# facebookresearch/momentum

Measured on AMD Instinct MI355X. Metric: character IK solves/sec (72-joint, 10 GN iters), higher is better.
Workload: dtype f32; 1 GPU; BASELINE configs[1]: B x 72-joint humanoid, P=128, pos+ori on 16 landmarks (M=192), GN lambda=0.05, 10 it; batch_per_gpu=4096, global_batch=4096, joints=72, params=128, rows=192, solved_parameters=96, route=fused, line_search=0, precision=f32

## Files before the change

### include/mmx.h

```cpp
#ifndef MMX_H_
#define MMX_H_

#include <stddef.h>
#include <stdint.h>

#ifdef __cplusplus
extern "C" {
#endif

#define MMX_ABI_VERSION 12
#define MMX_PARAMS_PER_JOINT 7
#define MMX_INVALID_PARENT (-1)
#define MMX_MAX_MODEL_PARAMS 2048

typedef enum mmx_status {
  MMX_OK = 0,
  MMX_ERR_INVALID_ARGUMENT = 1,
  MMX_ERR_SIZE_MISMATCH = 2,
  MMX_ERR_DEVICE = 3,
  MMX_ERR_UNSUPPORTED = 4,
  MMX_ERR_OUT_OF_MEMORY = 5,
  MMX_ERR_NO_DEVICE = 6
} mmx_status;

// ... 136 lines not shown

typedef struct mmx_rig mmx_rig;
typedef struct mmx_problem mmx_problem;

void mmx_gn_options_default(mmx_gn_options* opt);

int32_t mmx_abi_version(void);
const char* mmx_last_error(void);
int32_t mmx_device_count(void);

int32_t mmx_rig_create(const mmx_rig_desc* desc, int32_t device, mmx_rig** out);
void mmx_rig_destroy(mmx_rig* rig);
int32_t mmx_rig_num_joints(const mmx_rig* rig);
int32_t mmx_rig_num_params(const mmx_rig* rig);

int32_t mmx_problem_create(
    mmx_rig* rig,
    int32_t batch,
    int32_t num_pos,
    const int32_t* pos_parent,
    int32_t num_ori,
    const int32_t* ori_parent,
    mmx_problem** out);
void mmx_problem_destroy(mmx_problem* problem);

int32_t mmx_problem_set_instance_rig(
    mmx_problem* problem,
    const float* translation_offset,
    const float* pre_rotation,
    int32_t memory,
    void* stream);

int32_t mmx_problem_set_instance_parents(
    mmx_problem* problem,
    const int32_t* pos_parent,
    const int32_t* ori_parent,
    int32_t memory,
    void* stream);

#define MMX_ROUTE_AUTO 0
#define MMX_ROUTE_FUSED 1
#define MMX_ROUTE_WIDE 2
#define MMX_ROUTE_EXPLICIT_JACOBIAN 3
#define MMX_ROUTE_WAVE 4
#define MMX_WAVE_MAX_JOINTS 64
#define MMX_WAVE_MAX_SOLVED 32
#define MMX_WAVE_MAX_UNITS 192
typedef struct mmx_tuning {
  int32_t route;
  int32_t max_refinement_steps;
  float mixed_tolerance;
  int32_t mixed_max_cg;
  int32_t joint_pruning;
  int32_t reserved[3];
} mmx_tuning;
int32_t mmx_problem_set_tuning(mmx_problem* problem, const mmx_tuning* tuning);
int32_t mmx_problem_last_route(const mmx_problem* problem);
int32_t mmx_problem_num_solve_joints(const mmx_problem* problem);

int32_t mmx_problem_num_rows(const mmx_problem* problem);
int32_t mmx_problem_batch(const mmx_problem* problem);

int32_t mmx_problem_set_enabled(mmx_problem* problem, const uint8_t* enabled);

int32_t mmx_problem_set_constraints(
    mmx_problem* problem,
    const mmx_constraint_data* data,
    void* stream);
int32_t mmx_problem_set_constraints_sized(
    mmx_problem* problem,
    const mmx_constraint_data* data,
    size_t data_size,
    void* stream);

int32_t mmx_eval_jacobian(
    mmx_problem* problem,
    const float* theta_dev,
    float* jac_dev,
    float* res_dev,
    double* err_dev,
    int32_t layout,
    void* stream);

int32_t mmx_eval_jacobian_timed(
    mmx_problem* problem,
    const float* theta_dev,
    float* jac_dev,
    float* res_dev,
    double* err_dev,
    int32_t layout,
    void* stream,
    float* kernel_ms);

int32_t mmx_debug_store_pattern(mmx_problem* problem, float* jac_dev, void* stream, float* kernel_ms);

int32_t mmx_eval_skeleton_state(
    mmx_problem* problem,
    const float* theta_dev,
    float* state_dev,
    void* stream);

int32_t mmx_eval_normal_equations(
    mmx_problem* problem,
    const float* theta_dev,
    float* jtj_dev,
    float* jtr_dev,
    double* err_dev,
    void* stream);

int32_t mmx_solve(
    mmx_problem* problem,
// ... 148 lines not shown
```

### momentum_amd/_abi.py

```python
from __future__ import annotations

import ctypes as C

import numpy as np

c_float_p = C.POINTER(C.c_float)
c_double_p = C.POINTER(C.c_double)
c_int32_p = C.POINTER(C.c_int32)
c_uint8_p = C.POINTER(C.c_uint8)

MMX_ABI_VERSION = 12
MMX_OK = 0
MMX_SOLVE_OK, MMX_SOLVE_NONFINITE, MMX_SOLVE_NOT_PD = 0, 1, 2
MMX_SOLVE_DAMPING_FLOORED = 4
MMX_SOLVE_PRECISION_SUSPECT = 8
MMX_SOLVE_ESCALATED_F64 = 16
MMX_SOLVE_MIXED = 32
MMX_SOLVE_ERROR_MASK = 3
MMX_PRECISION_F32, MMX_PRECISION_F64, MMX_PRECISION_AUTO, MMX_PRECISION_MIXED = 0, 1, 2, 3
MMX_MEM_HOST, MMX_MEM_DEVICE = 0, 1
MMX_LAYOUT_COL_MAJOR, MMX_LAYOUT_ROW_MAJOR = 0, 1
MMX_STEP_GN_FIXED_LAMBDA, MMX_STEP_LM_SCHEDULE, MMX_STEP_TRUST_REGION = 0, 1, 2


# ... 249 lines not shown
        ("do_line_search", C.c_int32),
        ("step_rule", C.c_int32),
        ("lm_lambda_min", C.c_float),
        ("lm_lambda_max", C.c_float),
        ("lm_up", C.c_float),
        ("lm_down", C.c_float),
        ("trust_region_radius", C.c_float),
        ("precision", C.c_int32),
        ("precision_bound", C.c_float),
    ]

    @classmethod
    def make(
        cls,
        min_iterations=1,
        max_iterations=2,
        threshold=1.0,
        regularization=0.05,
        do_line_search=False,
        step_rule=MMX_STEP_GN_FIXED_LAMBDA,
        lm_lambda_min=1e-6,
        lm_lambda_max=1e6,
        lm_up=4.0,
        lm_down=0.5,
        trust_region_radius=1.0,
        precision=MMX_PRECISION_F32,
        precision_bound=1e-5,
    ) -> "GnOptions":
        return cls(
            int(min_iterations),
            int(max_iterations),
            float(threshold),
            float(regularization),
            int(do_line_search),
            int(step_rule),
            float(lm_lambda_min),
            float(lm_lambda_max),
            float(lm_up),
            float(lm_down),
            float(trust_region_radius),
            int(precision),
            float(precision_bound),
        )


ROUTES = {"auto": 0, "fused": 1, "wide": 2, "explicit_jacobian": 3, "wave": 4}
WAVE_MAX_JOINTS = 64
WAVE_MAX_SOLVED = 32
WAVE_MAX_UNITS = 192


class Tuning(C.Structure):

    _fields_ = [("route", C.c_int32), ("max_refinement_steps", C.c_int32), ("mixed_tolerance", C.c_float), ("mixed_max_cg", C.c_int32), ("joint_pruning", C.c_int32), ("reserved", C.c_int32 * 3)]


def as_ptr(a: np.ndarray, ctype):
    assert a.flags["C_CONTIGUOUS"], "array must be C-contiguous"
    return a.ctypes.data_as(C.POINTER(ctype))


def void_p(a) -> C.c_void_p:
    if a is None:
        return C.c_void_p(0)
    if isinstance(a, np.ndarray):
        assert a.flags["C_CONTIGUOUS"]
        return C.c_void_p(a.ctypes.data)
    return C.c_void_p(int(a))
```

### momentum_amd/build.py

```python
from __future__ import annotations

import os
import shutil
import subprocess
import sys

HERE = os.path.dirname(os.path.abspath(__file__))
CSRC = os.path.join(HERE, "csrc")
VARIANT = os.environ.get("MMX_BUILD_VARIANT", "")
VARIANT_FLAGS = os.environ.get("MMX_BUILD_FLAGS", "").split() if VARIANT else []
LIB = os.path.join(HERE, f"libmmx_hip_{VARIANT}.so" if VARIANT else "libmmx_hip.so")
SOURCES = ["mmx_kernels.hip", "mmx_fused.hip", "mmx_capi.hip", "mmx_comm.hip", "mmx_f64.hip", "mmx_host_tables.cpp", "mmx_solve_plan.cpp", "mmx_constraint_intake.cpp", "mmx_wave.hip", "mmx_wave_frames.hip", "mmx_gradient.hip"]
FUSED_GROUPS = 7
SOLVE_KERNEL_FLAGS = ["-mllvm", "-disable-machine-licm", "-mllvm", "-disable-lsr"]
BUILD_INFO = os.path.join(HERE, "build_info.json")
_probe_cache = {}


def solve_flags_accepted() -> bool:
    if os.environ.get("MMX_BUILD_DEFAULT_PIPELINE"):
        return False
    if "ok" not in _probe_cache:
        import tempfile

        with tempfile.TemporaryDirectory() as td:
            src = os.path.join(td, "probe.hip")
            with open(src, "w") as f:
                f.write("#include <hip/hip_runtime.h>\n__global__ void k(float* p) { for (int i = 0; i < 8; ++i) p[i * 3] += 1.f; }\n")
            cmd = [_hipcc(), f"--offload-arch={ARCH}", "-O3", "-c", src, "-o", os.path.join(td, "probe.o")] + SOLVE_KERNEL_FLAGS
            r = subprocess.run(cmd, stdout=subprocess.PIPE, stderr=subprocess.PIPE)
            _probe_cache["ok"] = r.returncode == 0
            if r.returncode != 0:
                print(
                    "WARNING momentum_amd/build.py: hipcc rejects " + " ".join(SOLVE_KERNEL_FLAGS) + " -- the solve kernels are built with the "
                    "DEFAULT pipeline (they spill vector registers and run 6-13 % slower; build_info.json says so):\n" + r.stderr.decode(errors="replace")[-400:],
                    file=sys.stderr,
                )
    return _probe_cache["ok"]


def _wants_solve_flags(src: str, group) -> bool:
    return src in ("mmx_f64.hip",) or (src == "mmx_fused.hip" and group != 4)


def _extra_flags(src: str, group) -> list:
    if _wants_solve_flags(src, group):
        return SOLVE_KERNEL_FLAGS
    return []


def build_info() -> dict:
    import json

    try:
        with open(BUILD_INFO) as f:
            return json.load(f)
    except (OSError, ValueError):
        return {}
SOURCE_DEPS = {"mmx_wave_frames.hip": ["mmx_wave.hip"]}
HEADERS = ["mmx_device.hpp", "mmx_device_d.hpp", "mmx_kernels.hpp", "mmx_tree.hpp", "mmx_fused_helpers.hpp", "mmx_host_tables.hpp", "mmx_solve_plan.hpp", "mmx_constraint_intake.hpp", os.path.join("..", "..", "include", "mmx.h")]
ARCH = "gfx950"


def _hipcc() -> str:
    for cand in (shutil.which("hipcc"), "/opt/rocm/bin/hipcc"):
        if cand and os.path.exists(cand):
            return cand
    raise RuntimeError("hipcc not found (ROCm toolchain required to build the gfx950 kernels)")


def needs_build() -> bool:
    if not os.path.exists(LIB) or (not VARIANT and not os.path.exists(BUILD_INFO)):
        return True
    t = os.path.getmtime(LIB)
    deps = [os.path.join(CSRC, s) for s in SOURCES + HEADERS]
    return any(os.path.getmtime(d) > t for d in deps)


def build(force: bool = False, verbose: bool = False) -> str:
    if not force and not needs_build():
        return LIB
    jobs, keep = [], []
    flags_ok = solve_flags_accepted()
    hdr_time = max(os.path.getmtime(os.path.join(CSRC, h)) for h in HEADERS)
    for src in SOURCES:
        groups = range(FUSED_GROUPS) if src == "mmx_fused.hip" else [None]
        for g in groups:
            stem = os.path.splitext(src)[0] + ("" if g is None else f"_g{g}")
            obj = os.path.join(CSRC, stem + (f".{VARIANT}" if VARIANT else "") + ".o")
            cmd = [_hipcc(), f"--offload-arch={ARCH}", "-O3", "-std=c++17", "-fPIC", "-c", os.path.join(CSRC, src), "-o", obj]
            if VARIANT:
                cmd.insert(1, f"-DMMX_EXP_{VARIANT.upper()}")
                cmd[1:1] = VARIANT_FLAGS
            if g is not None:
                cmd.insert(1, f"-DMMX_FUSED_GROUP={g}")
            if flags_ok:
                cmd[1:1] = _extra_flags(src, g)
            if src.endswith(".cpp"):
                cmd.insert(1, "-x")
                cmd.insert(2, "hip")
            src_time = max(os.path.getmtime(os.path.join(CSRC, d)) for d in [src] + SOURCE_DEPS.get(src, []))
            if not force and os.path.exists(obj) and os.path.getmtime(obj) > max(hdr_time, src_time):
                keep.append((None, obj))
                continue
            jobs.append((cmd, obj))
    from concurrent.futures import ThreadPoolExecutor

    def run(job):
        if verbose:
            print(" ".join(job[0]), file=sys.stderr)
        subprocess.check_call(job[0])
        return job[1]

# ... 35 lines not shown
```

### momentum_amd/capi.py

```python
from __future__ import annotations

import ctypes as C
import os
from typing import Optional

import numpy as np

from . import _abi
from ._abi import ConstraintData, GnOptions, RigDesc, as_ptr
from .rigs import Rig

_HERE = os.path.dirname(os.path.abspath(__file__))
LIB_PATH = os.environ.get("MMX_LIB") or os.path.join(_HERE, "libmmx_hip.so")
_lib: Optional[C.CDLL] = None

SYMBOLS = [
    "mmx_gn_options_default", "mmx_abi_version", "mmx_last_error", "mmx_device_count",
    "mmx_rig_create", "mmx_rig_destroy", "mmx_rig_num_joints", "mmx_rig_num_params",
    "mmx_problem_create", "mmx_problem_destroy", "mmx_problem_num_rows", "mmx_problem_batch",
    "mmx_problem_set_tuning", "mmx_problem_last_route", "mmx_problem_num_solve_joints",
    "mmx_problem_set_enabled", "mmx_problem_set_constraints", "mmx_problem_set_constraints_sized", "mmx_problem_set_instance_rig", "mmx_problem_set_instance_parents", "mmx_eval_jacobian", "mmx_eval_jacobian_timed", "mmx_debug_store_pattern",
    "mmx_eval_skeleton_state", "mmx_eval_normal_equations", "mmx_solve", "mmx_solve_with_history", "mmx_solve_with_step_history", "mmx_problem_solve_diagnostics", "mmx_solve_f64", "mmx_solve_f64_host", "mmx_solve_host",
    "mmx_solve_frames", "mmx_solve_frames_host",
    "mmx_eval_gradient", "mmx_eval_gradient_host",
    "mmx_eval_jacobian_host", "mmx_eval_skeleton_state_host", "mmx_host_tables", "mmx_debug_fused_normal_equations", "mmx_debug_tree_normal_equations",
    "mmx_host_elimination_order", "mmx_host_tile_structure", "mmx_host_tile_level_schedule", "mmx_host_f64_assembly_list", "mmx_problem_tile_structure", "mmx_host_live_joints",
    "mmx_comm_unique_id", "mmx_comm_create", "mmx_comm_create_all", "mmx_comm_world_size", "mmx_comm_rank",
    "mmx_comm_all_reduce_norms", "mmx_comm_all_reduce_norms_host", "mmx_residual_norms", "mmx_comm_destroy",
]


class MmxError(RuntimeError):

    def __init__(self, code: int, msg: str):
        super().__init__(f"mmx error {code}: {msg}")
        self.code = code


def lib() -> C.CDLL:
    global _lib
    if _lib is not None:
        return _lib
    if not os.path.exists(LIB_PATH):
        raise MmxError(-1, f"{LIB_PATH} is missing: build it with `python -m momentum_amd.build` (no CPU fallback exists)")
    try:
        import torch
    except Exception:
        pass
    L = C.CDLL(LIB_PATH)
    vp, i32 = C.c_void_p, C.c_int32
    L.mmx_last_error.restype = C.c_char_p
    L.mmx_gn_options_default.restype = None
    L.mmx_gn_options_default.argtypes = [C.POINTER(GnOptions)]
    L.mmx_rig_create.argtypes = [C.POINTER(RigDesc), i32, C.POINTER(vp)]
    L.mmx_rig_destroy.argtypes = [vp]
    L.mmx_rig_destroy.restype = None
    L.mmx_rig_num_joints.argtypes = [vp]
    L.mmx_rig_num_params.argtypes = [vp]
    L.mmx_problem_create.argtypes = [vp, i32, i32, _abi.c_int32_p, i32, _abi.c_int32_p, C.POINTER(vp)]
    L.mmx_problem_destroy.argtypes = [vp]
    L.mmx_problem_destroy.restype = None
    L.mmx_problem_num_rows.argtypes = [vp]
    L.mmx_problem_batch.argtypes = [vp]
    L.mmx_problem_set_enabled.argtypes = [vp, _abi.c_uint8_p]
    L.mmx_problem_set_tuning.argtypes = [vp, C.POINTER(_abi.Tuning)]
    L.mmx_problem_last_route.argtypes = [vp]
    L.mmx_problem_num_solve_joints.argtypes = [vp]
    L.mmx_problem_set_constraints.argtypes = [vp, C.POINTER(ConstraintData), vp]
    L.mmx_problem_set_constraints_sized.argtypes = [vp, C.POINTER(ConstraintData), C.c_size_t, vp]
    L.mmx_problem_set_instance_rig.argtypes = [vp, vp, vp, i32, vp]
    L.mmx_problem_set_instance_parents.argtypes = [vp, vp, vp, i32, vp]
    L.mmx_eval_jacobian.argtypes = [vp, vp, vp, vp, vp, i32, vp]
    L.mmx_eval_jacobian_timed.argtypes = [vp, vp, vp, vp, vp, i32, vp, C.POINTER(C.c_float)]
    L.mmx_debug_store_pattern.argtypes = [vp, vp, vp, C.POINTER(C.c_float)]
    L.mmx_eval_skeleton_state.argtypes = [vp, vp, vp, vp]
    L.mmx_eval_normal_equations.argtypes = [vp, vp, vp, vp, vp, vp]
    L.mmx_solve.argtypes = [vp, C.POINTER(GnOptions), vp, vp, vp, vp, vp, vp]
    L.mmx_solve_with_history.argtypes = [vp, C.POINTER(GnOptions), vp, vp, vp, vp, vp, vp, vp]
    L.mmx_solve_with_step_history.argtypes = [vp, C.POINTER(GnOptions), vp, vp, vp, vp, vp, vp, vp, vp]
    L.mmx_problem_solve_diagnostics.argtypes = [vp, vp, vp]
    L.mmx_solve_f64.argtypes = [vp, C.POINTER(GnOptions), vp, vp, vp, vp, vp, vp]
    L.mmx_solve_host.argtypes = [vp, C.POINTER(GnOptions), vp, vp, vp, vp]
    L.mmx_solve_f64_host.argtypes = [vp, C.POINTER(GnOptions), vp, vp, vp, vp]
    L.mmx_solve_frames.argtypes = [vp, C.POINTER(GnOptions), i32, vp, vp, vp, vp, vp, vp, vp]
    L.mmx_solve_frames_host.argtypes = [vp, C.POINTER(GnOptions), i32, vp, vp, vp, vp]
    L.mmx_eval_gradient.argtypes = [vp, vp, vp, vp, vp]
    L.mmx_eval_gradient_host.argtypes = [vp, vp, vp, vp]
    L.mmx_eval_jacobian_host.argtypes = [vp, vp, vp, vp, vp, i32]
    L.mmx_eval_skeleton_state_host.argtypes = [vp, vp, vp]
    L.mmx_debug_tree_normal_equations.argtypes = [vp, vp, vp, vp, vp]
    L.mmx_debug_fused_normal_equations.argtypes = [vp, vp, vp, vp, _abi.c_int32_p, _abi.c_int32_p, vp]
    L.mmx_comm_unique_id.argtypes = [vp]
    L.mmx_comm_create.argtypes = [vp, i32, i32, i32, C.POINTER(vp)]
    L.mmx_comm_create_all.argtypes = [i32, _abi.c_int32_p, C.POINTER(vp)]
    L.mmx_comm_world_size.argtypes = [vp]
    L.mmx_comm_rank.argtypes = [vp]
    L.mmx_comm_all_reduce_norms.argtypes = [vp, vp, vp]
    L.mmx_comm_all_reduce_norms_host.argtypes = [vp, vp]
    L.mmx_residual_norms.argtypes = [i32, vp, vp, vp, vp, vp]
    L.mmx_comm_destroy.argtypes = [vp]
    L.mmx_comm_destroy.restype = None
    L.mmx_host_tables.argtypes = [
        C.POINTER(RigDesc), _abi.c_uint8_p, _abi.c_int32_p, _abi.c_int32_p, _abi.c_int32_p,
        _abi.c_uint8_p, _abi.c_int32_p, _abi.c_int32_p,
    ]
    u32p, i64p = C.POINTER(C.c_uint32), C.POINTER(C.c_int64)
    L.mmx_host_elimination_order.argtypes = [C.POINTER(RigDesc), _abi.c_uint8_p, _abi.c_int32_p, _abi.c_int32_p]
    L.mmx_host_tile_structure.argtypes = [i32, _abi.c_uint8_p, u32p, u32p, i64p]
    L.mmx_host_tile_level_schedule.argtypes = [i32, _abi.c_uint8_p, C.POINTER(C.c_int32)]
    L.mmx_problem_tile_structure.argtypes = [vp, u32p, u32p, _abi.c_int32_p, _abi.c_int32_p, i64p]
    L.mmx_host_live_joints.argtypes = [C.POINTER(RigDesc), i32, _abi.c_int32_p, _abi.c_uint8_p, _abi.c_int32_p, _abi.c_int32_p]
    _lib = L
    return L


def _check(rc: int) -> None:
    if rc != 0:
        raise MmxError(rc, lib().mmx_last_error().decode("utf-8", "replace"))


# ... 117 lines not shown


default_route = "auto"


class Problem:

    def __init__(self, rig_handle: RigHandle, batch: int, pos_parent, ori_parent):
        import torch

        self.rh = rig_handle
        self.B = int(batch)
        self.P = rig_handle.rig.num_params
        self.J = rig_handle.rig.num_joints
        self.pos_parent = np.ascontiguousarray(pos_parent, dtype=np.int32).reshape(-1)
        self.ori_parent = np.ascontiguousarray(ori_parent, dtype=np.int32).reshape(-1)
        self.Kp, self.Ko = len(self.pos_parent), len(self.ori_parent)
        self.M = 3 * self.Kp + 9 * self.Ko
        self.n = self.P
        self.device = torch.device("cuda", rig_handle.device)
        self._h = C.c_void_p(0)
        self._keep = []
        _check(
            lib().mmx_problem_create(
                rig_handle._h, self.B, self.Kp, as_ptr(self.pos_parent, C.c_int32), self.Ko,
                as_ptr(self.ori_parent, C.c_int32), C.byref(self._h),
            )
        )
        self._prefer_wide = default_route == "prefer_wide"
        if default_route not in ("auto", "prefer_wide"):
            self.set_route(default_route)

    def close(self) -> None:
        if self._h:
            lib().mmx_problem_destroy(self._h)
            self._h = C.c_void_p(0)

    def __del__(self):
        try:
            self.close()
        except Exception:
            pass

    def set_route(self, route: str, max_refinement_steps: int = 0) -> None:
        self._prefer_wide = default_route == "prefer_wide" and route == "auto"
        self._set_tuning(route, max_refinement_steps)

    def _set_tuning(self, route: str, max_refinement_steps: int = 0) -> None:
        t = _abi.Tuning()
        t.route = _abi.ROUTES[route]
        t.max_refinement_steps = int(max_refinement_steps)
        t.mixed_tolerance, t.mixed_max_cg = getattr(self, "_mixed", (0.0, 0))
        t.joint_pruning = 0 if getattr(self, "_joint_pruning", True) else -1
        self._route_args = (route, int(max_refinement_steps))
        _check(lib().mmx_problem_set_tuning(self._h, C.byref(t)))

    def set_mixed(self, tolerance: float = 0.0, max_cg: int = 0) -> None:
        self._mixed = (float(tolerance), int(max_cg))
        self._set_tuning(*getattr(self, "_route_args", ("auto", 0)))

    def set_joint_pruning(self, on: bool = True) -> None:
        self._joint_pruning = bool(on)
        self._set_tuning(*getattr(self, "_route_args", ("auto", 0)))

    def num_solve_joints(self) -> int:
        return int(lib().mmx_problem_num_solve_joints(self._h))

    def last_route(self) -> str:
        r = int(lib().mmx_problem_last_route(self._h))
        return {v: k for k, v in _abi.ROUTES.items()}[r]

    def set_enabled(self, enabled) -> None:
        e = np.ascontiguousarray(enabled, dtype=np.uint8).reshape(-1)
        assert e.shape[0] == self.P
        _check(lib().mmx_problem_set_enabled(self._h, as_ptr(e, C.c_uint8)))
        self.n = int(np.count_nonzero(e))

    def set_constraints(
        self, pos_offset, pos_target, pos_weight, ori_offset, ori_target, ori_weight,
        pos_function_weight: float = 1.0, ori_function_weight: float = 1.0,
        limits=None, limit_function_weight: float = 1.0,
        model_target=None, model_weights=None, model_function_weight: float = 1.0,
        pos_loss=(2.0, 1.0), ori_loss=(2.0, 1.0), joint_blocks=None, ellipsoid_limits=None, function_weights=None,
    ) -> None:
        import torch

        arrs = [pos_offset, pos_target, pos_weight, ori_offset, ori_target, ori_weight]
        shapes = [(self.B, self.Kp, 3), (self.B, self.Kp, 3), (self.B, self.Kp), (self.B, self.Ko, 4), (self.B, self.Ko, 4), (self.B, self.Ko)]
        if model_target is not None:
            arrs += [model_target, model_weights]
            shapes += [(self.B, self.P), (self.B, self.P)]
        on_dev = all(isinstance(a, torch.Tensor) for a in arrs)
        keep, ptrs = [], []
        for a, shp in zip(arrs, shapes):
            if on_dev:
                assert a.is_cuda and a.dtype == torch.float32 and a.is_contiguous() and tuple(a.shape) == shp, (a.shape, shp)
                keep.append(a)
                ptrs.append(C.c_void_p(a.data_ptr() if a.numel() else 0))
            else:
                x = np.ascontiguousarray(a, dtype=np.float32).reshape(shp)
                keep.append(x)
                ptrs.append(C.c_void_p(x.ctypes.data if x.size else 0))
        if model_target is None:
            ptrs += [C.c_void_p(0), C.c_void_p(0)]
        fw_ptr, fw_cols = C.c_void_p(0), 0
        if function_weights is not None:
            if on_dev:
                assert function_weights.is_cuda and function_weights.dtype == torch.float32 and function_weights.is_contiguous() and function_weights.shape[0] == self.B
                keep.append(function_weights)
                fw_ptr, fw_cols = C.c_void_p(function_weights.data_ptr()), int(function_weights.shape[1])
            else:
                fwh = np.ascontiguousarray(function_weights, dtype=np.float32).reshape(self.B, -1)
                keep.append(fwh)
                fw_ptr, fw_cols = C.c_void_p(fwh.ctypes.data), int(fwh.shape[1])
        limits = list(limits) if limits else []
        larr = _abi.limit_array(limits)
# ... 330 lines not shown
```

### momentum_amd/csrc/mmx_capi.hip

```cpp
#include "../../include/mmx.h"

#include <hip/hip_runtime.h>

#include <dlfcn.h>

#include <cfloat>
#include <cmath>
#include <cstdio>
#include <cstdlib>
#include <cstring>
#include <algorithm>
#include <new>
#include <map>
#include <memory>
#include <numeric>
#include <string>
#include <vector>

#include "mmx_constraint_intake.hpp"
#include "mmx_host_tables.hpp"
#include "mmx_kernels.hpp"
#include "mmx_solve_plan.hpp"

namespace {
// ... 460 lines not shown
  d.numMultiCols = int32_t(cp.multi.size());
  d.numZeroCols = int32_t(cp.zero.size());
  mmx::FusedDev& fd = pb->fdev;
  fd.U = pb->U;
  fd.Kp = pb->Kp;
  fd.n = n;
  fd.nsrc = int32_t(st.slots.size());
  fd.slotBase = st.slotBase;
  fd.nnz = rig->ptOuter.back();
  fd.subSize = pb->dSubSize.as<int32_t>();
  fd.dfsJoint = pb->dDfsJoint.as<int32_t>();
  fd.loadedPos = pb->dLoadedPos.as<int32_t>();
  fd.numLoaded = int32_t(st.loadedPos.size());
  fd.unitJoint = pb->dUnitJoint.as<int32_t>();
  fd.posUnitStart = pb->dPosUnitStart.as<int32_t>();
  fd.posUnits = pb->dPosUnits.as<int32_t>();
  fd.solveList = pb->dSolveList.as<int32_t>();
  fd.srcStart = pb->dSrcStart.as<int32_t>();
  fd.srcs = pb->dSrcs.as<mmx::ColumnSourceDev>();
  fd.comb = pb->dComb.as<int32_t>();
  fd.numComb = int32_t(runs.comb.size() / 3);
  fd.numCells = runs.numCells;
  fd.gTerms = pb->dTerms.as<uint4>();
  fd.termRounds = int32_t(rounds);
  fd.gTerms16 = pb->dTerms16.as<uint4>();
  fd.termRounds16 = int32_t(rounds16);
  fd.pairCols = pb->dPairCols.as<int32_t>();
  fd.numLimits = int32_t(pb->limits.size());
  fd.limStart = pb->dLimStart.as<int32_t>();
  fd.limOf = pb->dLimOf.as<int32_t>();
  fd.numPairDests = int32_t(lt.pairDest.size());
  fd.pairDest = pb->dPairDest.as<int32_t>();
  fd.pairStart = pb->dPairStart.as<int32_t>();
  fd.pairLim = pb->dPairLim.as<int32_t>();
  fd.GT = G + NE;
  fd.genRows = fd.GT > 0 ? d.rowsJoint - 3 * pb->U : 0;
  fd.tileList = pb->dTileList.as<int32_t>();
  fd.numTiles = int32_t(pb->tileMasks.tiles.size());
  pb->viewBuilt = false;
  return wantView ? uploadSolveView(pb, lv) : MMX_OK;
}

struct SolveView {
  mmx::RigDev rig;
  mmx::ProblemDev pb;
  mmx::FusedDev fd;
};
bool solveViewActive(const mmx_problem* pb) {
  return pb->viewBuilt && pb->tuning.joint_pruning == 0 && pb->rigDev.instPreRot == nullptr && pb->rigDev.instOffset == nullptr &&
      pb->dev.instPosParent == nullptr && pb->dev.instOriParent == nullptr;
}
SolveView solveView(const mmx_problem* pb) {
  SolveView v{pb->rigDev, pb->dev, pb->fdev};
  if (!solveViewActive(pb)) {
    return v;
  }
  v.rig = pb->vRig;
  v.pb.unitJoint = pb->vUnitJoint.as<int32_t>();
  v.pb.unitTin = pb->vUnitTin.as<int32_t>();
  v.pb.jointTin = pb->vJointTin.as<int32_t>();
  v.pb.genJoint = pb->vGenJoint.as<int32_t>();
  v.pb.genTin = pb->vGenTin.as<int32_t>();
  v.pb.ellipsoids = pb->vEllipsoids.as<mmx::EllipsoidDev>();
  v.pb.limits = pb->vLimits.as<mmx::LimitDev>();
  v.fd.nnz = pb->vNnz;
  v.fd.subSize = pb->vSubSize.as<int32_t>();
  v.fd.dfsJoint = pb->vDfsJoint.as<int32_t>();
  v.fd.loadedPos = pb->vLoadedPos.as<int32_t>();
  v.fd.unitJoint = pb->vUnitJoint.as<int32_t>();
  v.fd.posUnitStart = pb->vPosUnitStart.as<int32_t>();
  v.fd.srcs = pb->vSrcs.as<mmx::ColumnSourceDev>();
  return v;
}

bool fusedUsable(const mmx_problem* pb) {
  const int nb = mmx::fusedBlocksFor(pb->fdev.n);
  if (nb < 0) {
    return false;
  }
  return pb->rig->J < 4096 &&
      mmx::fusedLdsBytes(nb, pb->rig->J, pb->rig->P, pb->U, pb->fdev.nsrc, pb->fdev.n, pb->fdev.numCells, true, pb->fdev.GT, pb->fdev.genRows, true, mmx::fusedCsrFloats(pb->rig->J, pb->fdev.nnz)) +
          size_t(8) * size_t(pb->rig->J + pb->rig->P) <=
      160 * 1024;
}

bool treeNormalEquationsUsable(const mmx_problem* pb) {
  return pb->U > 0 && pb->fdev.n > 0 && pb->fdev.n <= 512 && pb->fdev.nsrc < 4096 &&
      pb->fused.solveList == pb->solveListV1 &&
      mmx::treeNormalEquationsLdsBytes(pb->rig->J, pb->rig->P, pb->U, pb->fdev.nsrc, pb->fdev.n, pb->fdev.GT, pb->fdev.genRows) <= 160 * 1024 - 64 &&
      mmx::treeRefineLdsBytes(pb->rig->J, pb->rig->P, pb->U, pb->fdev.n, pb->fdev.genRows) <= 160 * 1024 - 64;
}

int32_t refineSteps(const mmx_problem* pb) {
  const int32_t m = pb->tuning.max_refinement_steps;
  return m == 0 ? 3 : (m < 0 ? 0 : (m > 3 ? 3 : m));
}

bool phaseClocksWanted() {
  static const bool wanted = getenv("MMX_PHASE_CLOCKS") != nullptr;
  return wanted;
}

hipError_t armPhaseStop(long long* clk, hipStream_t s) {
  static const long long stop = getenv("MMX_PHASE_STOP") != nullptr ? atoll(getenv("MMX_PHASE_STOP")) + 1 : 0;
  return stop > 0 ? hipMemcpyAsync(clk + 31, &stop, sizeof(long long), hipMemcpyHostToDevice, s) : hipSuccess;
}
// ... 410 lines not shown
    pb->posParent.assign(pos_parent, pos_parent + num_pos);
  }
  if (num_ori > 0) {
    pb->oriParent.assign(ori_parent, ori_parent + num_ori);
  }
  pb->tables = rig->topo;
  pb->rigDev = rig->dev;
  pb->dev.wPos = 1.f;
  pb->dev.wOri = 1.f;
  const int32_t rc = uploadProblemTables(pb);
  if (rc != MMX_OK) {
    delete pb;
    return rc;
  }
  *out = pb;
  return MMX_OK;
}

void mmx_problem_destroy(mmx_problem* pb) {
  if (pb != nullptr) {
    if (pb->rig != nullptr) {
      (void)hipSetDevice(pb->rig->device);
    }
    delete pb;
  }
}

int32_t mmx_problem_num_rows(const mmx_problem* pb) {
  return pb ? pb->M : 0;
}
int32_t mmx_problem_batch(const mmx_problem* pb) {
  return pb ? pb->B : 0;
}

int32_t mmx_problem_set_tuning(mmx_problem* pb, const mmx_tuning* tuning) {
  int32_t rc = checkProblem(pb, false);
  if (rc != MMX_OK) {
    return rc;
  }
  if (tuning == nullptr) {
    return fail(MMX_ERR_INVALID_ARGUMENT, "tuning is null");
  }
  if (tuning->route < MMX_ROUTE_AUTO || tuning->route > MMX_ROUTE_WAVE) {
    return fail(MMX_ERR_INVALID_ARGUMENT, "mmx_tuning::route: unknown MMX_ROUTE_* value");
  }
  if (tuning->max_refinement_steps < -1 || tuning->max_refinement_steps > 3) {
    return fail(MMX_ERR_INVALID_ARGUMENT, "mmx_tuning::max_refinement_steps: -1 (none), 0 (default) or 1..3");
  }
  if (!(tuning->mixed_tolerance >= 0.f) || tuning->mixed_tolerance > 1e-2f || tuning->mixed_max_cg < 0 || tuning->mixed_max_cg > 64) {
    return fail(MMX_ERR_INVALID_ARGUMENT, "mmx_tuning::mixed_tolerance: 0 (default) or (0, 1e-2]; mixed_max_cg: 0 (default) or 1..64");
  }
  if (tuning->joint_pruning != 0 && tuning->joint_pruning != -1) {
    return fail(MMX_ERR_INVALID_ARGUMENT, "mmx_tuning::joint_pruning: 0 (on) or -1 (off)");
  }
  for (int32_t r : tuning->reserved) {
    if (r != 0) {
      return fail(MMX_ERR_INVALID_ARGUMENT, "mmx_tuning::reserved must be zero");
    }
  }
  pb->tuning = *tuning;
  return MMX_OK;
}

int32_t mmx_problem_last_route(const mmx_problem* pb) {
  return pb != nullptr ? pb->lastRoute : MMX_ROUTE_AUTO;
}

int32_t mmx_problem_num_solve_joints(const mmx_problem* pb) {
  if (pb == nullptr || pb->rig == nullptr) {
    return 0;
  }
  return solveViewActive(pb) ? pb->liveJoints.numLive : pb->rig->J;
}

int32_t mmx_problem_set_enabled(mmx_problem* pb, const uint8_t* enabled) {
  MMX_ZONE("mmx_problem_set_enabled");
  int32_t rc = checkProblem(pb, false);
  if (rc != MMX_OK) {
    return rc;
  }
  if (enabled == nullptr) {
    return fail(MMX_ERR_INVALID_ARGUMENT, "enabled is null");
  }
  if (!pb->tablesDirty && pb->tables.enabled.size() == size_t(pb->rig->P)) {
    bool same = true;
    for (size_t p = 0; p < pb->tables.enabled.size() && same; ++p) {
      same = (pb->tables.enabled[p] != 0) == (enabled[p] != 0);
    }
    if (same) {
      return MMX_OK;
    }
  }
  const mmx_rig_desc d = pb->rig->desc();
  std::string err;
  mmx::HostTables t;
  rc = mmx::buildHostTables(&d, enabled, t, err);
  if (rc != MMX_OK) {
    return fail(rc, err);
  }
  pb->tables = std::move(t);
  return uploadProblemTables(pb);
}

int32_t mmx_problem_set_instance_rig(mmx_problem* pb, const float* translation_offset, const float* pre_rotation, int32_t memory, void* stream) {
  MMX_ZONE("mmx_problem_set_instance_rig");
  int32_t rc = checkProblem(pb, false);
// ... 885 lines not shown
  return rc;
}

int32_t solveImpl(mmx_problem* pb, const mmx_gn_options* o, float* theta_dev, const SolveOutputs& out, void* stream) {
  MMX_ZONE("mmx_solve (SolverT::solve)");
  if (o != nullptr) {
    if (const char* why = mmx::preHandleRefusal(*o, out.stepHistory != nullptr)) {
      return fail(MMX_ERR_INVALID_ARGUMENT, why);
    }
  }
  MMX_TRY(checkProblem(pb, true));
  if (o == nullptr || theta_dev == nullptr) {
    return fail(MMX_ERR_INVALID_ARGUMENT, "options / theta is null");
  }
  const mmx::SolvePlan plan = mmx::planSolve(solveFacts(pb, out, o->precision, pb->tuning.route == MMX_ROUTE_WAVE), *o);
  if (plan.code != MMX_OK) {
    return fail(plan.code, plan.message);
  }
  MMX_HIP(hipSetDevice(pb->rig->device));
  return runPlan(pb, o, plan, theta_dev, out, static_cast<hipStream_t>(stream));
}

template <typename T, typename Solve>
int32_t solveStaged(mmx_problem* pb, T* theta_host, double* final_error_host, int32_t* iterations_host, int32_t* status_host, Solve solve) {
  MMX_TRY(checkProblem(pb, true));
  if (theta_host == nullptr) {
    return fail(MMX_ERR_INVALID_ARGUMENT, "theta is null");
  }
  const size_t B = size_t(pb->B), P = size_t(pb->rig->P);
  MMX_HIP(hipSetDevice(pb->rig->device));
  MMX_HIP(pb->sTheta.ensure(B * P * sizeof(T)));
  MMX_HIP(pb->sIters.ensure(B * sizeof(int32_t)));
  MMX_HIP(pb->sStatus.ensure(B * sizeof(int32_t)));
  MMX_HIP(pb->sFinalErr.ensure(B * sizeof(double)));
  MMX_HIP(hipMemcpy(pb->sTheta.p, theta_host, B * P * sizeof(T), hipMemcpyHostToDevice));
  MMX_TRY(solve(pb->sTheta.as<T>(), pb->sFinalErr.as<double>(), pb->sIters.as<int32_t>(), pb->sStatus.as<int32_t>()));
  MMX_HIP(hipDeviceSynchronize());
  MMX_HIP(hipMemcpy(theta_host, pb->sTheta.p, B * P * sizeof(T), hipMemcpyDeviceToHost));
  if (final_error_host) {
    MMX_HIP(hipMemcpy(final_error_host, pb->sFinalErr.p, B * sizeof(double), hipMemcpyDeviceToHost));
  }
  if (iterations_host) {
    MMX_HIP(hipMemcpy(iterations_host, pb->sIters.p, B * sizeof(int32_t), hipMemcpyDeviceToHost));
  }
  if (status_host) {
    MMX_HIP(hipMemcpy(status_host, pb->sStatus.p, B * sizeof(int32_t), hipMemcpyDeviceToHost));
  }
  return MMX_OK;
}

}
}

int32_t mmx_solve(
    mmx_problem* pb,
    const mmx_gn_options* o,
    float* theta_dev,
    double* final_error,
    int32_t* iterations,
    int32_t* status,
    double* error_history,
    void* stream) {
  return solveImpl(pb, o, theta_dev, SolveOutputs{final_error, iterations, status, error_history, nullptr, nullptr}, stream);
}

int32_t mmx_solve_with_history(
    mmx_problem* pb,
    const mmx_gn_options* o,
    float* theta_dev,
    double* final_error,
    int32_t* iterations,
    int32_t* status,
    double* error_history,
    float* parameter_history,
    void* stream) {
  return solveImpl(pb, o, theta_dev, SolveOutputs{final_error, iterations, status, error_history, parameter_history, nullptr}, stream);
}

int32_t mmx_solve_with_step_history(
    mmx_problem* pb,
    const mmx_gn_options* o,
    float* theta_dev,
    double* final_error,
    int32_t* iterations,
    int32_t* status,
    double* error_history,
    float* parameter_history,
    double* step_history,
    void* stream) {
  return solveImpl(pb, o, theta_dev, SolveOutputs{final_error, iterations, status, error_history, parameter_history, step_history}, stream);
}

int32_t mmx_solve_f64(
    mmx_problem* pb,
    const mmx_gn_options* o,
    double* theta_dev,
    double* final_error,
    int32_t* iterations,
    int32_t* status,
    double* error_history,
    void* stream) {
  if (theta_dev == nullptr) {
    return fail(MMX_ERR_INVALID_ARGUMENT, "options / theta is null");
  }
  MMX_TRY(checkProblem(pb, true));
  if (o == nullptr) {
// ... 219 lines not shown
```

### momentum_amd/csrc/mmx_device.hpp

```cpp
#pragma once

#include <hip/hip_runtime.h>

#include <cstdint>

#include "../../include/mmx.h"
#include "mmx_constraint_intake.hpp"

namespace mmx {

constexpr int kJs = 17;
constexpr float kPivotFloor = 3.814697265625e-6f;
constexpr float kFactorDamping = 1e-5f;
constexpr float kPrecisionGain = 0.042f;
constexpr float kPivotFloorOrOne = kPivotFloor > 0.f ? kPivotFloor : 1.f;

constexpr float kLn2 = 0.693147180559945309417232121458176568f;

struct F3 {
  float x, y, z;
};
struct Q4 {
  float x, y, z, w;
};

__device__ __forceinline__ F3 f3(float x, float y, float z) {
  return F3{x, y, z};
}
__device__ __forceinline__ F3 operator+(F3 a, F3 b) {
  return F3{a.x + b.x, a.y + b.y, a.z + b.z};
}
__device__ __forceinline__ F3 operator-(F3 a, F3 b) {
  return F3{a.x - b.x, a.y - b.y, a.z - b.z};
}
__device__ __forceinline__ F3 operator*(float s, F3 a) {
  return F3{s * a.x, s * a.y, s * a.z};
}
__device__ __forceinline__ F3 cross(F3 a, F3 b) {
  return F3{a.y * b.z - a.z * b.y, a.z * b.x - a.x * b.z, a.x * b.y - a.y * b.x};
}
__device__ __forceinline__ float dot(F3 a, F3 b) {
  return a.x * b.x + a.y * b.y + a.z * b.z;
}
__device__ __forceinline__ Q4 qmul(Q4 a, Q4 b) {
  return Q4{
      a.w * b.x + a.x * b.w + a.y * b.z - a.z * b.y,
      a.w * b.y + a.y * b.w + a.z * b.x - a.x * b.z,
      a.w * b.z + a.z * b.w + a.x * b.y - a.y * b.x,
      a.w * b.w - a.x * b.x - a.y * b.y - a.z * b.z};
}
__device__ __forceinline__ F3 qrot(Q4 q, F3 v) {
  const F3 qv{q.x, q.y, q.z};
  F3 uv = cross(qv, v);
  uv = uv + uv;
  return v + q.w * uv + cross(qv, uv);
}
__device__ __forceinline__ F3 qmatCol(Q4 q, int c) {
  const float tx = 2.f * q.x, ty = 2.f * q.y, tz = 2.f * q.z;
  const float twx = tx * q.w, twy = ty * q.w, twz = tz * q.w;
  const float txx = tx * q.x, txy = ty * q.x, txz = tz * q.x;
  const float tyy = ty * q.y, tyz = tz * q.y, tzz = tz * q.z;
  if (c == 0) {
    return F3{1.f - (tyy + tzz), txy + twz, txz - twy};
  }
// ... 174 lines not shown
}
__device__ __forceinline__ JointBlockDev jointBlockOf(const ProblemDev& pb, int b, int i) {
  JointBlockDev k = pb.blocks[i];
  if (pb.fnWeights != nullptr && 4 + i < pb.fnCols) {
    k.fw *= pb.fnWeights[size_t(b) * size_t(pb.fnCols) + size_t(4 + i)];
  }
  return k;
}
__device__ __forceinline__ int jointBlockSecondJoint(const ProblemDev& pb, const JointBlockDev& k, int g) {
  return k.type == MMX_JC_JOINT_TO_JOINT_DISTANCE ? pb.genJoint[pb.G + g] : -1;
}
__device__ __forceinline__ int jointBlockSecondTin(const ProblemDev& pb, const JointBlockDev& k, int g) {
  return k.type == MMX_JC_JOINT_TO_JOINT_DISTANCE ? pb.genTin[pb.G + g] : -1;
}

__device__ __forceinline__ void
fkLocalFromParams(const float* jpv, const float* pre, const float* off, float* o, float* oq) {
  float sx, cx, sy, cy, sz, cz;
  sincosf(0.5f * jpv[3], &sx, &cx);
  sincosf(0.5f * jpv[4], &sy, &cy);
  sincosf(0.5f * jpv[5], &sz, &cz);
  const Q4 q0{pre[0], pre[1], pre[2], pre[3]};
  const Q4 q1 = qmul(q0, Q4{0.f, 0.f, sz, cz});
  const Q4 q2 = qmul(q1, Q4{0.f, sy, 0.f, cy});
  const Q4 ql = qmul(q2, Q4{sx, 0.f, 0.f, cx});
  o[0] = off[0] + jpv[0], o[1] = off[1] + jpv[1], o[2] = off[2] + jpv[2];
  o[3] = ql.x, o[4] = ql.y, o[5] = ql.z, o[6] = ql.w;
  o[7] = exp2f(jpv[6]);
  oq[0] = q1.x, oq[1] = q1.y, oq[2] = q1.z, oq[3] = q1.w;
  oq[4] = q2.x, oq[5] = q2.y, oq[6] = q2.z, oq[7] = q2.w;
}

template <class RigT>
__device__ __forceinline__ void
fkLocalSplit(const RigT& rig, int j, const float* __restrict__ theta, float* o, float* oq) {
  float jpv[7];
#pragma unroll
  for (int d = 0; d < 7; ++d) {
    const int r = 7 * j + d;
    float acc = 0.f;
    const int k1 = rig.ptOuter[r + 1];
    for (int k = rig.ptOuter[r]; k < k1; ++k) {
      acc += rig.ptValue[k] * theta[rig.ptInner[k]];
    }
    jpv[d] = acc + rig.ptOffsets[r];
  }
  fkLocalFromParams(jpv, rig.preRot + 4 * j, rig.offset + 3 * j, o, oq);
}
template <class RigT>
__device__ __forceinline__ void fkLocalTo(const RigT& rig, int j, const float* __restrict__ theta, float* o) {
  fkLocalSplit(rig, j, theta, o, o + 8);
}

constexpr int kFkCh = 9;
__host__ __device__ __forceinline__ int fkPad(int J) {
  return (J + 1) & ~1;
}
__host__ __device__ __forceinline__ size_t fkBufFloats(int J) {
  return 2 * size_t(kFkCh) * size_t(fkPad(J));
}
struct FkXf {
  double tx, ty, tz, qx, qy, qz, qw, s;
  int jl;
};
__device__ __forceinline__ FkXf fkLoadD(const double* buf, int Jp, int j) {
  FkXf x;
  x.tx = buf[j], x.ty = buf[Jp + j], x.tz = buf[2 * Jp + j];
  x.qx = buf[3 * Jp + j], x.qy = buf[4 * Jp + j], x.qz = buf[5 * Jp + j], x.qw = buf[6 * Jp + j];
  x.s = buf[7 * Jp + j];
  x.jl = reinterpret_cast<const int*>(buf + 8 * Jp)[2 * j];
  return x;
}
__device__ __forceinline__ void fkStoreD(double* buf, int Jp, int j, const FkXf& x) {
  buf[j] = x.tx, buf[Jp + j] = x.ty, buf[2 * Jp + j] = x.tz;
  buf[3 * Jp + j] = x.qx, buf[4 * Jp + j] = x.qy, buf[5 * Jp + j] = x.qz, buf[6 * Jp + j] = x.qw;
  buf[7 * Jp + j] = x.s;
  reinterpret_cast<int*>(buf + 8 * Jp)[2 * j] = x.jl;
}
__device__ __forceinline__ void fkStoreLocalD(double* bufA, int Jp, int j, const float* o, int parentPlus1) {
  FkXf x;
  x.tx = o[0], x.ty = o[1], x.tz = o[2], x.qx = o[3], x.qy = o[4], x.qz = o[5], x.qw = o[6];
  x.s = o[7], x.jl = parentPlus1;
  fkStoreD(bufA, Jp, j, x);
}
__device__ __forceinline__ void fkComposeD(const FkXf& p, FkXf& x) {
  const double sp = p.s;
  const double vx = sp * x.tx, vy = sp * x.ty, vz = sp * x.tz;
  double ux = p.qy * vz - p.qz * vy, uy = p.qz * vx - p.qx * vz, uz = p.qx * vy - p.qy * vx;
  ux += ux, uy += uy, uz += uz;
  const double tx = p.tx + (vx + p.qw * ux + (p.qy * uz - p.qz * uy));
  const double ty = p.ty + (vy + p.qw * uy + (p.qz * ux - p.qx * uz));
  const double tz = p.tz + (vz + p.qw * uz + (p.qx * uy - p.qy * ux));
  const double qx = p.qw * x.qx + p.qx * x.qw + p.qy * x.qz - p.qz * x.qy;
  const double qy = p.qw * x.qy + p.qy * x.qw + p.qz * x.qx - p.qx * x.qz;
  const double qz = p.qw * x.qz + p.qz * x.qw + p.qx * x.qy - p.qy * x.qx;
  const double qw = p.qw * x.qw - p.qx * x.qx - p.qy * x.qy - p.qz * x.qz;
  x.tx = tx, x.ty = ty, x.tz = tz, x.qx = qx, x.qy = qy, x.qz = qz, x.qw = qw;
  x.s = p.s * x.s;
  x.jl = p.jl;
}
template <class T, int kStride = kJs>
__device__ __forceinline__ void fkJumpRoundsT(T* js, double* bufA, double* bufB, int J, int rounds, int tid, int nthreads) {
  const int Jp = fkPad(J);
  for (int r = 0; r < rounds; ++r) {
    const double* src = (r & 1) ? bufB : bufA;
    double* dst = (r & 1) ? bufA : bufB;
    const bool last = r == rounds - 1;
    for (int j = tid; j < J; j += nthreads) {
      FkXf x = fkLoadD(src, Jp, j);
      const int a = x.jl - 1;
      if (a >= 0) {
        const FkXf p = fkLoadD(src, Jp, a);
        fkComposeD(p, x);
// ... 560 lines not shown
    }
    if (o.idx[0] == o.idx[1]) {
      o.idx[0] = -1;
      o.coef[0] = T(0);
    }
    o.err = tWeight * T(lm.weight) * (rs * rs);
  } else if (lm.type == 4) {
    bool actRef, actTgt;
    const T jr = limitJointParam(rig, th, enabled, lm.index0, actRef);
    const T jt = limitJointParam(rig, th, enabled, lm.index1, actTgt);
    const float jtF = float(jt);
    const bool inRange = (lm.v[2] == 0.f && lm.v[3] == 0.f) || (jtF >= lm.v[2] && jtF < lm.v[3]);
    if ((!actRef && !actTgt) || !inRange) {
      return o;
    }
    const T rs = jt * T(lm.v[0]) - T(lm.v[1]) - jr;
    o.r = rs * wgt;
    if (actTgt) {
      limitScatterRow(rig, o, lm.index1, T(lm.v[0]) * wgt);
    }
    if (actRef) {
      limitScatterRow(rig, o, lm.index0, -wgt);
    }
    o.err = tWeight * T(lm.weight) * (rs * rs);
  } else if (lm.type == 6) {
    const int p1 = lm.index0, p2 = lm.index1;
    if (!enabled[p1] && !enabled[p2]) {
      return o;
    }
    const T rs = th[p1] * T(lm.v[0]) + th[p2] * T(lm.v[1]) - T(lm.v[2]);
    if (rs >= T(0)) {
      return o;
    }
    o.r = rs * wgt;
    if (enabled[p1]) {
      o.idx[0] = p1;
      o.coef[0] = T(lm.v[0]) * wgt;
    }
    if (enabled[p2]) {
      o.idx[1] = p2;
      o.coef[1] = T(lm.v[1]) * wgt;
    }
    if (o.idx[0] == o.idx[1]) {
      o.idx[0] = -1;
      o.coef[0] = T(0);
    }
    o.err = tWeight * T(lm.weight) * (rs * rs);
  }
  return o;
}

typedef float v4f __attribute__((ext_vector_type(4)));

constexpr int kTan = 9;

__device__ __forceinline__ int tileAddr(int row, int col) {
  return row * 16 + ((((col >> 2) ^ (row >> 2)) & 3) << 2) + (col & 3);
}
__device__ __forceinline__ int tileIndex(int I, int Jc) {
  return I * (I + 1) / 2 + Jc;
}
__device__ __forceinline__ void tileDecode(int t, int& I, int& Jc) {
  int i = int((sqrtf(8.f * float(t) + 1.f) - 1.f) * 0.5f);
  while ((i + 1) * (i + 2) / 2 <= t) {
    ++i;
  }
  while (i * (i + 1) / 2 > t) {
    --i;
  }
  I = i;
  Jc = t - i * (i + 1) / 2;
}

__device__ __forceinline__ float readLaneF(float v, int lane) {
  return __int_as_float(__builtin_amdgcn_readlane(__float_as_int(v), lane));
}

typedef float v2f __attribute__((ext_vector_type(2)));
__device__ __forceinline__ void panelRowUpdate1(float (&a)[16], int j) {
#pragma unroll
  for (int c = j + 1; c < 16; ++c) {
    a[c] -= a[j] * readLaneF(a[j], c);
  }
}
__device__ __forceinline__ void panelRowUpdate(float (&a)[16], int j) {
  if ((j & 1) == 0) {
    a[j + 1] -= a[j] * readLaneF(a[j], j + 1);
  }
#pragma unroll
  for (int c = (j + 2) & ~1; c < 16; c += 2) {
    const v2f mlt{readLaneF(a[j], c), readLaneF(a[j], c + 1)};
    const v2f aj2{a[j], a[j]};
    v2f acc{a[c], a[c + 1]};
    acc = __builtin_elementwise_fma(-aj2, mlt, acc);
    a[c] = acc.x, a[c + 1] = acc.y;
  }
}

__device__ __forceinline__ float4 ldsRow4(const float* tile, int row, int chunk) {
  return *reinterpret_cast<const float4*>(tile + row * 16 + (((chunk ^ (row >> 2)) & 3) << 2));
}
__device__ __forceinline__ float dot4pk(float4 a, float4 b, float acc) {
  v2f s{acc, 0.f};
  s = __builtin_elementwise_fma(v2f{a.x, a.y}, v2f{b.x, b.y}, s);
  s = __builtin_elementwise_fma(v2f{a.z, a.w}, v2f{b.z, b.w}, s);
  return s.x + s.y;
}
// ... 80 lines not shown
```

### momentum_amd/csrc/mmx_fused.hip

```cpp
#include "mmx_device.hpp"
#include "mmx_fused_helpers.hpp"
#include "mmx_kernels.hpp"
#include "mmx_mixed.hpp"
#include "mmx_tree.hpp"

#include <cfloat>
#include <cstdlib>

namespace mmx {

struct MixRowRec {
  int4 q{0, 0, 0, 0};
  bool has = false;
};
template <typename Gather, typename Store>
__device__ __forceinline__ void mixTransformRows(const RigView& rig, int tid, Gather x, Store out, const MixRowRec& regRec = MixRowRec{}) {
  if (regRec.has) {
    if (tid < rig.numRowRec) {
      const int4 q = regRec.q;
      const int row = q.x & 0xffff, span = int(uint32_t(q.x) >> 16), in0 = q.y & 0xffff, cnt = int(uint32_t(q.y) >> 16);
      auto acc = __int_as_float(q.z) * x(in0);
      for (int k = q.w + 1; k < q.w + cnt; ++k) {
        acc += rig.ptValue[k] * x(rig.ptInner[k]);
      }
// ... 196 lines not shown
  __syncthreads();
  for (int r = 0; r < rig.jumpRounds; ++r) {
    int next = -1;
    if (target >= 0) {
      const double* t = m.Y + kTanD * target;
#pragma unroll
      for (int c = 0; c < 7; ++c) {
        acc[c] += t[c];
      }
      next = reinterpret_cast<const int*>(t + 7)[0];
    }
    __syncthreads();
    if (target >= 0) {
      double* o = m.Y + kTanD * tid;
#pragma unroll
      for (int c = 0; c < 7; ++c) {
        o[c] = acc[c];
      }
      reinterpret_cast<int*>(o + 7)[0] = next;
    }
    target = next;
    __syncthreads();
  }
}

template <class FV>
__device__ __forceinline__ void mixApply(
    const RigView& rig, const FV& fd, const FusedLds& s, const MixLds& m, const int16_t* parentPos, int J, int NP, int n, int nsrc, double mu, const double* p, double* q, int tid, const MixRowRec& regRec = MixRowRec{}) {
  mixTangent(
      rig, fd, m, parentPos, J, tid,
      [&](int c) {
        const int cs = fd.colToSolve[c];
        return cs >= 0 ? p[cs] : 0.0;
      },
      regRec);
  mixAdjoint(
      fd, s, m, J, NP, n, nsrc, tid,
      [&](int u, int k, const D3& pu) {
        const double* pre = m.Y + kTanD * k;
        D3 v = dcross(D3{pre[3], pre[4], pre[5]}, pu);
        if (u < fd.Kp) {
          v = D3{pre[0], pre[1], pre[2]} + v + (kLn2D * pre[6]) * pu;
        }
        const double sg = m.us[u];
        return (sg * sg) * v;
      },
      q);
  for (int c = tid; c < n; c += 256) {
    q[c] += mu * p[c];
  }
  __syncthreads();
}

constexpr int kGenEv = 29;

template <int NB, bool kTR, bool kGen, int kRule>
struct FusedFour {
  static constexpr bool value = NB <= 6 && !kGen && !kTR;
};

struct FusedLayout {
  size_t uyFloats;
  size_t auxOff;
  size_t cellOff;
  size_t t9;
  size_t arenaFloats;
  size_t umomFloats;
  size_t regionFloats;
  size_t genFloats;
  size_t total;
};
__host__ __device__ inline FusedLayout fusedLayout(int NB, int J, int P, int U, int nsrc, int n, int numCells, bool cellsBehindRho, int GT, int genRows, bool separateUy = false, size_t csrFloats = 0, bool mix = false) {
  auto a4 = [](size_t x) { return (x + 3) & ~size_t(3); };
  auto h4 = [&](size_t x) { return a4((x + 1) / 2); };
  auto mx = [](size_t x, size_t y) { return x > y ? x : y; };
  const size_t T = size_t(NB) * (NB + 1) / 2, NP = 16 * size_t(NB);
  FusedLayout l;
  l.cellOff = cellsBehindRho ? 2 * NP : 0;
  const size_t aux = a4(mx(2 * NP, mx(size_t(nsrc), l.cellOff + size_t(numCells))));
  l.auxOff = separateUy ? a4(3 * size_t(U)) : 0;
  l.uyFloats = separateUy ? l.auxOff + aux : mx(a4(3 * size_t(U)), aux);
  l.t9 = a4(size_t(kTan) * J);
  l.arenaFloats = mx(size_t(kSrcCh - 1) * size_t(srcStrideFor(nsrc)), 2 * l.t9 + a4(P));
  if (mix) {
    l.arenaFloats = mx(size_t(kSrcCh - 1) * size_t(srcStrideFor(nsrc)), a4(2 * (mixXDoubles(J, nsrc) + mixYDoubles(J, P))));
  }
  l.umomFloats = mx(a4(size_t(kUmom) * U), a4(size_t(kC1) * J));
  const size_t scratch = fkBufFloats(J) + 2 * a4(size_t(kC2) * J) + l.umomFloats;
  l.regionFloats = mx(scratch, T * 256);
  const size_t rowsGp = a4(size_t(genRows));
  l.genFloats = GT > 0 ? a4(size_t(kGenEv) * GT) + 2 * a4(rowsGp) + a4(rowsGp * size_t(srcStrideFor(int(NP)))) : 0;
  const size_t meta = h4(NP + 1) + 3 * a4(nsrc) + a4(J) + 4 * h4(J) + h4(size_t(J) + 1) + 2 * h4(U) + h4(n) + h4(P);
  size_t fixed = a4(P) + a4(size_t(kJs) * J) + 2 * a4(3 * size_t(U)) + a4(U) + 2 * a4(NP) + l.uyFloats + 16 + 8;
  if (mix) {
    fixed = l.uyFloats + 40 + 8 + a4(2 * mixPersistentDoubles(J, P, U, int(NP))) + 2 * h4(J);
  }
  l.total = meta + fixed + l.genFloats + l.arenaFloats + l.regionFloats + csrFloats;
  return l;
}

__device__ __forceinline__ double generalRowsError(const ProblemDev& pb, const float* js, int b, int tid) {
  double e = 0.0;
  for (int g = tid; g < pb.G; g += 256) {
    const JointBlockDev k = jointBlockOf(pb, b, pb.genBlock[g]);
    e += double(evalJointConstraint(k, js, pb.genJoint[g], jointBlockSecondJoint(pb, k, g), size_t(b) * size_t(k.count) + size_t(g - k.first)).werr);
  }
  if (pb.wLimit > 0.f) {
    const float tWeightE = 1e+1f * pb.wLimit;
    for (int q = tid; q < pb.NE; q += 256) {
      e += double(evalEllipsoid(pb.ellipsoids[q], js, tWeightE).werr);
    }
  }
  return e;
}

__device__ __forceinline__ double generalRowsEvaluate(const ProblemDev& pb, const float* js, int b, int U, int tid, float* gEv, float* gRes) {
  double e = 0.0;
  int* evi = reinterpret_cast<int*>(gEv);
  for (int g = tid; g < pb.G; g += 256) {
    const JointBlockDev k = jointBlockOf(pb, b, pb.genBlock[g]);
    const int i = g - k.first;
    const JointEval o = evalJointConstraint(k, js, pb.genJoint[g], jointBlockSecondJoint(pb, k, g), size_t(b) * size_t(k.count) + size_t(i));
    const int row = k.rowStart + o.nrows * i - 3 * U;
    e += double(o.werr);
    for (int q = 0; q < o.nrows; ++q) {
      gRes[row + q] = o.sigma * o.f[q];
    }
    const float sg = fabsf(o.sigma) <= 1e-9f ? 0.f : o.sigma;
    float* w = gEv + kGenEv * g;
    w[0] = o.vp.x, w[1] = o.vp.y, w[2] = o.vp.z;
    w[3] = o.vn.x, w[4] = o.vn.y, w[5] = o.vn.z;
#pragma unroll
    for (int q = 0; q < 9; ++q) {
      w[6 + q] = sg * o.dp[q];
      w[15 + q] = sg * o.dn[q];
    }
    evi[kGenEv * g + 24] = pb.genTin[g];
    evi[kGenEv * g + 25] = row;
    evi[kGenEv * g + 26] = jointEvalFlags(o);
    evi[kGenEv * g + 27] = jointBlockSecondTin(pb, k, g);
  }
  const float tWeightE = 1e+1f * pb.wLimit;
  for (int q = tid; q < pb.NE; q += 256) {
    const EllipsoidDev ct = pb.ellipsoids[q];
    const int row = pb.rowsJoint - 3 * pb.NE + 3 * q - 3 * U, g = pb.G + q;
    EllipsoidEval o = evalEllipsoid(ct, js, tWeightE);
    if (!(pb.wLimit > 0.f)) {
      o.jwgt = o.werr = 0.f;
    }
    e += double(o.werr);
    gRes[row] = o.diff.x * o.jwgt, gRes[row + 1] = o.diff.y * o.jwgt, gRes[row + 2] = o.diff.z * o.jwgt;
// ... 38 lines not shown
      const float* a = js + kJs * sl.joint;
      F3 gp{0.f, 0.f, 0.f}, gn{0.f, 0.f, 0.f};
      if (sl.dof >= 3 && sl.dof < 6) {
        const float* ax = a + 8 + 3 * (sl.dof - 3);
        const F3 axis{ax[0], ax[1], ax[2]};
        if (hasPoint) {
          gp = cross(axis, vp - F3{a[0], a[1], a[2]});
        }
        if (hasDir) {
          gn = cross(axis, vn);
        }
      } else if (hasPoint) {
        gp = sl.dof < 3 ? transAxisCol(js, sl.parent, sl.dof) : kLn2 * (vp - F3{a[0], a[1], a[2]});
      }
#pragma unroll
      for (int q = 0; q < 3; ++q) {
        const float jc = (w[6 + 3 * q] * gp.x + w[7 + 3 * q] * gp.y + w[8 + 3 * q] * gp.z) +
            (w[15 + 3 * q] * gn.x + w[16 + 3 * q] * gn.y + w[17 + 3 * q] * gn.z);
        acc[q] += jc * sl.weight;
      }
    };
    auto addSlotPair = [&](int e) {
      const GenSlot sl = slot(e);
      const bool anc = sl.tin <= tin && tin < sl.tout, anc2 = sl.tin <= tinStop && tinStop < sl.tout;
      if (!anc && !anc2) {
        return;
      }
      const F3 gd = pairSourceDerivative(js, sl.joint, sl.dof, anc, anc2, vp, vn, [&]() { return transAxisCol(js, sl.parent, sl.dof); });
      acc[0] += (w[6] * gd.x + w[7] * gd.y + w[8] * gd.z) * sl.weight;
    };
    int e0, e1;
    extras(c, e0, e1);
    if ((fl & 64) != 0) {
      addSlotPair(c);
      for (int e = e0; e < e1; ++e) {
        addSlotPair(e);
      }
    } else {
      addSlot(c);
      for (int e = e0; e < e1; ++e) {
        addSlot(e);
      }
    }
    gJ[row * gst + c] = acc[0];
    if ((fl & 15) >= 2) {
      gJ[(row + 1) * gst + c] = acc[1];
    }
    if ((fl & 15) == 3) {
      gJ[(row + 2) * gst + c] = acc[2];
    }
  }
}

template <bool kGen = false, bool kStore = false, bool kGlobalCsr = true, class FV = FusedViewS>
__device__ __forceinline__ double blockError(
    const RigDev& rigDev,
    const RigView& rig,
    const ProblemDev& pb,
    const FV& fd,
    const FusedLds& s,
    const float* th,
    int b,
    int tid,
    double* unrounded = nullptr) {
  const int lane = tid & 63, wave = tid >> 6;
  blockFk<kGlobalCsr>(rig, s, th, tid, kStore);
  double e = 0.0;
  for (int u = tid; u < fd.U; u += 256) {
    const Unit un = evalUnit(pb, s.js, b, u);
    if (kStore) {
      s.up[3 * u] = un.v.x, s.up[3 * u + 1] = un.v.y, s.up[3 * u + 2] = un.v.z;
      const float rx = un.sigma * un.f.x, ry = un.sigma * un.f.y, rz = un.sigma * un.f.z;
      s.ur[3 * u] = rx, s.ur[3 * u + 1] = ry, s.ur[3 * u + 2] = rz;
      s.uy[3 * u] = un.sigma * rx, s.uy[3 * u + 1] = un.sigma * ry, s.uy[3 * u + 2] = un.sigma * rz;
      s.us[u] = un.sigma;
    }
    e += double(un.werr);
  }
  if (pb.M > pb.rowsJoint) {
    e += paramRowsError<false>(rigDev, pb, rig.P, th, b, tid);
  }
  if (kGen) {
    e += generalRowsError(pb, s.js, b, tid);
  }
  e = waveReduceSum(e);
  if (lane == 0) {
    s.red[wave] = e;
  }
  __syncthreads();
  const double tot = (s.red[0] + s.red[1]) + (s.red[2] + s.red[3]);
  __syncthreads();
  if (unrounded != nullptr) {
    *unrounded = tot;
  }
  return double(float(tot));
}

__device__ __forceinline__ float blockSumF(const FusedLds& s, float v, int tid) {
  v = waveReduceSumF(v);
  if ((tid & 63) == 0) {
    s.red[4 + (tid >> 6)] = double(v);
  }
  __syncthreads();
  const float tot = float((s.red[4] + s.red[5]) + (s.red[6] + s.red[7]));
  __syncthreads();
  return tot;
}

__device__ __forceinline__ float quadSum(float v) {
  v += __int_as_float(__builtin_amdgcn_update_dpp(0, __float_as_int(v), 0xB1, 0xF, 0xF, true));
  v += __int_as_float(__builtin_amdgcn_update_dpp(0, __float_as_int(v), 0x4E, 0xF, 0xF, true));
  return v;
}

template <int NB>
__device__ __forceinline__ void solveLLtLeft(const float* L, const float* invDiag, float* x, int tid) {
  if (tid < 64) {
    const int i = tid >> 2, g = tid & 3;
#pragma unroll
    for (int k = 0; k < NB; ++k) {
      float acc = 0.f;
#pragma unroll
// ... 381 lines not shown
  static_assert(!kMix || (!kTR && !kGen && kRule == -1 && !kArgLazy), "the mixed-precision instantiation: generic rule, reference rows");
  constexpr int T = NB * (NB + 1) / 2;
  constexpr int NP = 16 * NB;
  constexpr bool kLook = NB <= 8;
  long long clkLast = 0;
  const int dbgStop = (MODE == 2 && dbgClk != nullptr) ? int(dbgClk[31]) : 0;
#define MMX_CLK(slot)                                             \
  if (MODE == 2 && blockIdx.x == 0 && threadIdx.x == 0) {         \
    const long long now_ = clock64();                             \
    dbgClk[slot] += now_ - clkLast;                               \
    clkLast = now_;                                               \
  }                                                               \
  if (MODE == 2 && dbgStop == (slot) + 1) {                       \
    __builtin_amdgcn_endpgm();                                    \
  }
  extern __shared__ __attribute__((aligned(16))) float smem[];
  int bSel = blockIdx.x;
  if (kMix && sel.map != nullptr) {
    if (int(blockIdx.x) >= *sel.count) {
      return;
    }
    bSel = sel.map[blockIdx.x];
  }
  const int b = bSel, tid = threadIdx.x;
  const int wave = tid >> 6, lane = tid & 63;
  RigDev rigV;
  ProblemDev pbV;
  if (!kArgLazy) {
    rigV = rigArg;
    pbV = pbArg;
    selectInstanceRig(rigV, b);
    selectInstanceWeights(pbV, b);
  }
  const RigDev& rig = kArgLazy ? argsDev->rig : rigV;
  const ProblemDev& pb = kArgLazy ? argsDev->pb : pbV;
  const FusedDev& fd = kArgLazy ? argsDev->fd : fdV;
  const SolveStateDev& st = kArgLazy ? argsDev->st : stV;
  const FusedParams& fp = kArgLazy ? argsDev->fp : fpV;
  const int J = rig.J, P = rig.P, U = fd.U, n = fd.n, nsrc = fd.nsrc;
  const int JL = rig.layoutJ;
  const int kR = rig.R;

  FusedLds s;
  int16_t *lParentPos, *lSubSize, *lPosUnitStart, *lPosUnits, *lUnitJoint, *lSolveList, *lDfsJoint, *lLoadedPos, *lColToSolve;
  int *lParent, *lPtOuter = nullptr, *lPtInner = nullptr;
  float *srcGu, *cells, *arena, *lPtValue = nullptr;
  constexpr bool kFour = FusedFour<NB, kTR, kGen, kRule>::value && !kMix;
  constexpr bool kCsrLds = !kFour && !kMix;
  constexpr bool kLeanSolve = kFour;
  constexpr bool kRide = kFour && NB >= 2;
  constexpr bool kLeanOps = kFour;
  constexpr bool kLeanAcc = kFour;
  const int kNnz = fd.nnz;
  const FusedLayout lay = fusedLayout(NB, JL, P, U, nsrc, n, fd.numCells, kRule < 0, kGen ? fd.GT : 0, kGen ? fd.genRows : 0, kTR, 0, kMix);
  MixLds m{};
  m.layoutJ = JL;
  {
    float* p = smem;
    auto take = [&](size_t count) {
      float* r = p;
      p += alignUp4(count);
      return r;
    };
    auto takeS = [&](size_t count) { return reinterpret_cast<int16_t*>(take((count + 1) / 2)); };
    s.mStart = takeS(NP + 1);
    s.mTin = reinterpret_cast<int*>(take(nsrc));
    s.mInfo = reinterpret_cast<int*>(take(nsrc));
    s.mW = take(nsrc);
    lParent = reinterpret_cast<int*>(take(JL));
    lParentPos = takeS(JL);
    lSubSize = takeS(JL);
    lPosUnitStart = takeS(JL + 1);
    lPosUnits = takeS(U);
    lUnitJoint = takeS(U);
    lSolveList = takeS(n);
    lDfsJoint = takeS(JL);
    lLoadedPos = takeS(JL);
    lColToSolve = takeS(P);
    if (kCsrLds) {
      lPtOuter = reinterpret_cast<int*>(take(kR + 1));
      lPtInner = reinterpret_cast<int*>(take(kNnz));
      lPtValue = take(kNnz);
    }
    if (kMix) {
      s.th = s.js = s.up = s.us = s.ur = s.g = s.d0 = nullptr;
      m.lo = takeS(JL);
      m.hi = takeS(JL);
    } else {
      s.th = take(P);
      s.js = take(size_t(kJs) * JL);
      s.up = take(3 * size_t(U));
      s.ur = take(3 * size_t(U));
      s.us = take(U);
      s.g = take(NP);
      s.d0 = take(NP);
    }
    s.uy = take(lay.uyFloats);
    s.rho = s.uy + lay.auxOff, s.invDiag = s.rho + NP, srcGu = s.rho, cells = s.rho + lay.cellOff;
    s.red = reinterpret_cast<double*>(take(kMix ? 40 : 16));
    s.flags = reinterpret_cast<int*>(take(8));
    s.gEv = s.gRes = s.gW = s.gJ = nullptr;
    if (kGen) {
      const int rowsGp = (fd.genRows + 3) & ~3;
      s.gEv = take(size_t(kGenEv) * size_t(fd.GT));
      s.gRes = take(rowsGp);
      s.gW = take(rowsGp);
      s.gJ = take(size_t(rowsGp) * size_t(srcStrideFor(NP)));
    }
    arena = take(lay.arenaFloats);
    if (kMix) {
      m.X = reinterpret_cast<double*>(arena);
      m.Y = m.X + mixXDoubles(JL, nsrc);
    }
    s.srcT = arena;
    s.tanOwn = arena, s.jd = arena + lay.t9, s.tanPre = arena + lay.t9, s.dfull = arena + 2 * lay.t9;
    float* region = p;
    s.fkA = reinterpret_cast<double*>(take(fkBufFloats(JL)));
    s.fkB = reinterpret_cast<double*>(p);
    s.own2 = take(size_t(kC2) * JL);
    s.sub2 = take(size_t(kC2) * JL);
    s.umom = take(lay.umomFloats);
    s.own1 = region, s.sub1 = s.umom;
    s.L = region;
    if (kMix) {
      double* d = reinterpret_cast<double*>(smem + (lay.total - alignUp4(2 * mixPersistentDoubles(JL, P, U, NP))));
      m.th = d, d += P;
      m.js = d, d += size_t(kJsD) * JL;
      m.up = d, d += 3 * size_t(U);
      m.uf = d, d += 3 * size_t(U);
      m.us = d, d += U;
      m.g = d, d += NP;
      m.x = d, d += NP;
      m.r = d, d += NP;
      m.p = d, d += NP;
      m.q = d;
    }
  }

  float* thg = theta + size_t(b) * P;
  if (kMix) {
    const float* th0 = sel.thetaInit != nullptr ? sel.thetaInit + size_t(b) * P : thg;
    for (int i = tid; i < P; i += 256) {
      m.th[i] = double(th0[i]);
    }
  } else {
    for (int i = tid; i < P; i += 256) {
      s.th[i] = thg[i];
    }
  }
  for (int c = tid; c <= NP; c += 256) {
    s.mStart[c] = int16_t(fd.srcStart[c]);
  }
  for (int e = tid; e < nsrc; e += 256) {
    const ColumnSourceDev cs = fd.srcs[e];
    s.mTin[e] = cs.tin | (cs.tout << 16);
    s.mInfo[e] = cs.joint | (cs.dof << 12) | ((cs.parent + 1) << 16);
    s.mW[e] = cs.weight;
  }
  for (int i = tid; i < J; i += 256) {
    lParent[i] = rig.parent[i];
    lSubSize[i] = int16_t(fd.subSize[i]);
  }
  for (int i = tid; i <= J; i += 256) {
    lPosUnitStart[i] = int16_t(fd.posUnitStart[i]);
  }
  if (kCsrLds) {
    for (int i = tid; i <= kR; i += 256) {
      lPtOuter[i] = rig.ptOuter[i];
    }
    for (int i = tid; i < kNnz; i += 256) {
      lPtInner[i] = rig.ptInner[i];
      lPtValue[i] = rig.ptValue[i];
    }
  }
  for (int i = tid; i < U; i += 256) {
    lPosUnits[i] = int16_t(fd.posUnits[i]);
    lUnitJoint[i] = int16_t(pb.unitTin[i]);
  }
  for (int i = tid; i < n; i += 256) {
    lSolveList[i] = int16_t(fd.solveList[i]);
  }
  for (int i = tid; i < J; i += 256) {
    lDfsJoint[i] = int16_t(fd.dfsJoint[i]);
    lLoadedPos[i] = int16_t(i < fd.numLoaded ? fd.loadedPos[i] : 0);
  }
  for (int i = tid; i < P; i += 256) {
    lColToSolve[i] = -1;
  }
  if (kGen) {
    const int rowsGp = (fd.genRows + 3) & ~3;
    for (int i = tid; i < rowsGp * srcStrideFor(NP); i += 256) {
      s.gJ[i] = 0.f;
    }
    for (int i = tid; i < rowsGp; i += 256) {
      s.gRes[i] = 0.f;
      s.gW[i] = 0.f;
    }
  }
  __syncthreads();
  for (int i = tid; i < n; i += 256) {
    lColToSolve[fd.solveList[i]] = int16_t(i);
  }
  int numLoadedInst = fd.numLoaded;
  if (pb.instPosParent != nullptr || pb.instOriParent != nullptr) {
    __syncthreads();
    numLoadedInst = buildInstanceUnitTables(pb, fd, b, J, U, tid, lUnitJoint, lPosUnitStart, lPosUnits, lLoadedPos);
  }
  {
    int* posOf = reinterpret_cast<int*>(s.fkA);
    for (int k = tid; k < J; k += 256) {
      posOf[fd.dfsJoint[k]] = k;
    }
    __syncthreads();
    for (int k = tid; k < J; k += 256) {
      const int par = rig.parent[fd.dfsJoint[k]];
      lParentPos[k] = int16_t(par >= 0 ? posOf[par] : -1);
    }
  }
  RigView rv;
  rv.J = J, rv.P = P, rv.R = kR, rv.numLevels = rig.numLevels, rv.jumpRounds = rig.jumpRounds;
  rv.parent = lParent, rv.preRot = asGlobal(rig.preRot), rv.offset = asGlobal(rig.offset);
  rv.ptOuter = kCsrLds ? lPtOuter : asGlobal(rig.ptOuter), rv.ptInner = kCsrLds ? lPtInner : asGlobal(rig.ptInner), rv.ptValue = kCsrLds ? lPtValue : asGlobal(rig.ptValue);
  rv.ptOffsets = asGlobal(rig.ptOffsets);
  rv.hasOffsets = rig.ptOffsetsNonZero != 0;
  rv.levelOrder = nullptr, rv.levelStart = nullptr;
  rv.rowRec = asGlobal(rig.ptRowRec), rv.numRowRec = rig.numRowRec;
  FusedViewS fv;
  fv.U = U, fv.Kp = fd.Kp;
  fv.dfsJoint = lDfsJoint, fv.loadedPos = lLoadedPos, fv.numLoaded = numLoadedInst, fv.colToSolve = lColToSolve;
  fv.subSize = lSubSize, fv.unitPos = lUnitJoint, fv.posUnitStart = lPosUnitStart, fv.posUnits = lPosUnits;
  fv.solveList = lSolveList;
  float* estAcc = reinterpret_cast<float*>(s.flags + 4);
  if (tid == 0) {
    s.flags[0] = 0;
    s.flags[1] = 0;
    s.flags[2] = 0;
    estAcc[0] = estAcc[1] = 0.f, estAcc[2] = -1.f;
  }
  int4 mixRec{0, 0, 0, 0};
  const bool mixHasRec = kMix && rv.rowRec != nullptr && rv.numRowRec <= 256;
  if (mixHasRec && tid < rv.numRowRec) {
    mixRec = rv.rowRec[tid];
  }
  const MixRowRec mixRecP{mixRec, mixHasRec};
  int mixLevel = 0;
  if (kMix && tid < J) {
    for (int a = lParent[tid]; a >= 0; a = lParent[a]) {
      ++mixLevel;
    }
  }
  if (kMix) {
    for (int k = tid; k < J; k += 256) {
      const int end = k + lSubSize[k];
      int lo = 0, hi = 0;
      for (int li = 0; li < numLoadedInst; ++li) {
        const int pp = lLoadedPos[li];
        lo += pp < k ? 1 : 0;
        hi += pp < end ? 1 : 0;
      }
      m.lo[k] = int16_t(lo), m.hi[k] = int16_t(hi);
    }
  }
  const bool hasParamRows = kRule >= 0 ? false : (pb.M > pb.rowsJoint);
  double lastError = DBL_MAX;
  float lambda = fp.lambda;
  double lambdaD = double(fp.lambda);
  bool mixUnconverged = false;
  int mixApplied = 0;
  float trRadius = fp.trustRadius;
  double curError = DBL_MAX;
  int itersDone = 0;
  float pivotWorst = 0.f;
  float refineWorst = 0.f;
  constexpr bool kReuse = !kGen && !kTR && kRule != 0;
  const int stepRule = kRule < 0 ? fp.stepRule : (kRule == 1 ? 1 : 0);
  const int doLineSearch = kRule < 0 || kRule == 2 ? fp.doLineSearch : 0;
  bool stateValid = false;
  double stateError = 0.0;
  __syncthreads();

  if (MODE == 2) {
    clkLast = clock64();
  }
  const int tidOuter = tid;
  for (int it = 0; it < fp.maxIterations; ++it) {
    int tid = tidOuter;
    asm volatile("" : "+v"(tid));
    const int lane = tid & 63;
    const int wave = __builtin_amdgcn_readfirstlane(tid >> 6);
    constexpr bool kLateUnit = kFour || kMix;
    const UnitInput uin0 = kLateUnit ? UnitInput{} : loadUnitInput(pb, b, tid < U ? tid : U);
    float trLambda = 1e-10f;
    int trustStep = 0;
    bool trNoStep = false;
    float trDn2 = 0.f, trDg = 0.f, trMu = 0.f;
    bool notPd = false;
    bool badPivot = false;
    bool floored = false;
    for (;;) {
    int tidT = tid;
    if (kTR) {
      asm volatile("" : "+v"(tidT));
    }
    {
    const int tid = tidT;
    const int lane = tid & 63;
    const int wave = __builtin_amdgcn_readfirstlane(tid >> 6);
    if (kReuse && stateValid) {
      curError = stateError;
    } else if (kMix) {
      blockFkD(rv, m, m.th, tid, mixLevel, true, mixRecP);
      double e = mixUnits<true>(pb, s, m, b, U, tid);
      if (hasParamRows) {
        e += paramRowsErrorD<true>(rig, pb, P, m.th, b, tid);
      }
      e = waveReduceSum(e);
      if (lane == 0) {
        s.red[wave] = e;
      }
      __syncthreads();
      curError = (s.red[0] + s.red[1]) + (s.red[2] + s.red[3]);
      MMX_CLK(1)
    } else {
    blockFk<!kCsrLds>(rv, s, s.th, tid, true, MODE == 2 ? dbgClk : nullptr, &clkLast);
    MMX_CLK(1)
    {
      double e = 0.0;
      for (int u = tid; u < U; u += 256) {
        const Unit un = evalUnitFrom(pb, (!kLateUnit && u == tid) ? uin0 : loadUnitInput(pb, b, u), s.js, u);
        s.up[3 * u] = un.v.x, s.up[3 * u + 1] = un.v.y, s.up[3 * u + 2] = un.v.z;
        const float rx = un.sigma * un.f.x, ry = un.sigma * un.f.y, rz = un.sigma * un.f.z;
        s.ur[3 * u] = rx, s.ur[3 * u + 1] = ry, s.ur[3 * u + 2] = rz;
        s.uy[3 * u] = un.sigma * rx, s.uy[3 * u + 1] = un.sigma * ry, s.uy[3 * u + 2] = un.sigma * rz;
        s.us[u] = un.sigma;
        e += double(un.werr);
      }
      if (hasParamRows) {
        e += paramRowsError<true>(rig, pb, P, s.th, b, tid);
      }
      if (kGen) {
        e += generalRowsEvaluate(pb, s.js, b, U, tid, s.gEv, s.gRes);
      }
      e = waveReduceSum(e);
      if (lane == 0) {
        s.red[wave] = e;
      }
    }
    __syncthreads();
    curError = (s.red[0] + s.red[1]) + (s.red[2] + s.red[3]);
    }
    if (kGen) {
      generalRowsGather(
          s.js, s.gEv, s.gJ, srcStrideFor(NP), fd.GT, n, tid,
          [&](int e) {
            const int span = s.mTin[e], info = s.mInfo[e];
            return GenSlot{span & 0xffff, span >> 16, info & 0xfff, (info >> 12) & 7, (info >> 16) - 1, s.mW[e]};
          },
          [&](int c, int& e0, int& e1) { e0 = NP + s.mStart[c], e1 = NP + s.mStart[c + 1]; });
      __syncthreads();
    }
    MMX_CLK(2)
    if (kMix) {
      __syncthreads();
      mixAdjoint(
          fv, s, m, J, NP, n, nsrc, tid,
          [&](int u, int, const D3&) {
            const double sg = m.us[u];
            return (sg * sg) * D3{m.uf[3 * u], m.uf[3 * u + 1], m.uf[3 * u + 2]};
          },
          m.g);
      __syncthreads();
      MMX_CLK(5)
    }
    int newtonIter = 0, pdRetries = 0;
    for (;;) {
    int tidS = tid;
    if (kTR) {
      asm volatile("" : "+v"(tidS));
    }
    {
    const int tid = tidS;
    const int lane = tid & 63;
// ... 550 lines not shown
        }
        __syncthreads();
#pragma unroll
        for (int q = 0; q < 5; ++q) {
          sums[q] = (s.red[4 * q] + s.red[4 * q + 1]) + (s.red[4 * q + 2] + s.red[4 * q + 3]);
        }
        __syncthreads();
        const double am2 = alpha > 1.0 ? alpha * alpha : 1.0;
        if (am2 * sums[4] * am2 * sums[4] <= tol2 * sums[1] * sums[0]) {
          for (int c = tid; c < n; c += 256) {
            m.x[c] += double(s.rho[c]);
          }
          converged = true;
        } else {
          const double beta = -alpha * sums[3] / rz;
          for (int c = tid; c < n; c += 256) {
            m.p[c] = double(s.rho[c]) + beta * m.p[c];
          }
          rz = sums[2];
          converged = !(rz > 0.0);
          if (k >= 5 && am2 * sums[4] > 1e-6 * sums[1]) {
            __syncthreads();
            break;
          }
        }
        __syncthreads();
        MMX_CLK(18)
      }
      mixUnconverged = mixUnconverged || !converged;
    } else if (kRide) {
      solveLLtAheadTail<NB>(s.L, s.invDiag, s.d0, tid);
    } else if (!notPd) {
      solveLLt<NB, kLeanSolve>(s.L, s.invDiag, s.d0, tid);
    }
    MMX_CLK(8)
    const int nRefine = (!notPd && !kMix) ? fp.refine : 0;
    float prevCorr2 = FLT_MAX;
    for (int rf = 0; rf < nRefine; ++rf) {
      {
        auto xd = [&](int c) {
          const int cs = fv.colToSolve[c];
          return cs >= 0 ? s.d0[cs] : 0.f;
        };
        auto od = [&](int r, float a) { s.jd[r] = a; };
        if (kCsrLds) {
          for (int r = tid; r < rv.R; r += 256) {
            float a = 0.f;
            const int k1 = rv.ptOuter[r + 1];
            for (int k = rv.ptOuter[r]; k < k1; ++k) {
              a += rv.ptValue[k] * xd(rv.ptInner[k]);
            }
            od(r, a);
          }
        } else if (rv.rowRec != nullptr) {
          csrRowsFromRecords<256>(rv.rowRec, rv.numRowRec, rv.ptInner, rv.ptValue, rv.R, tid, xd, od);
        } else {
          csrRowsPrefetched<256>(rv.ptOuter, rv.ptInner, rv.ptValue, rv.R, tid, xd, od);
        }
      }
      __syncthreads();
      MMX_CLK(16)
      if (kGen) {
        const int gst = srcStrideFor(NP);
        for (int r = tid; r < fd.genRows; r += 256) {
          float a = s.gRes[r];
          for (int c = 0; c < n; ++c) {
            a -= s.gJ[r * gst + c] * s.d0[c];
          }
          s.gW[r] = a;
        }
      }
      for (int k = tid; k < J; k += 256) {
        const int q = fv.dfsJoint[k];
        const float* ja = s.js + kJs * q;
        const float* d = s.jd + 7 * q;
        const F3 ta{ja[0], ja[1], ja[2]};
        F3 Tv{0.f, 0.f, 0.f};
        if (d[0] != 0.f || d[1] != 0.f || d[2] != 0.f) {
          const int par = rv.parent[q];
          Tv = d[0] * transAxisCol(s.js, par, 0) + d[1] * transAxisCol(s.js, par, 1) + d[2] * transAxisCol(s.js, par, 2);
        }
        const F3 Om = d[3] * F3{ja[8], ja[9], ja[10]} + d[4] * F3{ja[11], ja[12], ja[13]} + d[5] * F3{ja[14], ja[15], ja[16]};
        const F3 C = Tv - cross(Om, ta) - (kLn2 * d[6]) * ta;
        float* o = s.tanOwn + kTan * k;
        o[0] = C.x, o[1] = C.y, o[2] = C.z, o[3] = Om.x, o[4] = Om.y, o[5] = Om.z, o[6] = d[6], o[7] = 0.f;
      }
      __syncthreads();
      if (JL <= 256) {
        float acc[7];
        int target = -1;
        if (tid < J) {
#pragma unroll
          for (int c = 0; c < 7; ++c) {
            acc[c] = s.tanOwn[kTan * tid + c];
          }
          target = lParentPos[tid];
          s.tanPre[kTan * tid + 7] = __int_as_float(target);
#pragma unroll
          for (int c = 0; c < 7; ++c) {
            s.tanPre[kTan * tid + c] = acc[c];
          }
        }
        __syncthreads();
        for (int r = 0; r < rv.jumpRounds; ++r) {
          int next = -1;
          if (target >= 0) {
// ... 232 lines not shown
          lambdaD = fmax(lambdaD * double(fp.lmDown), double(fp.lmLambdaMin));
        }
        lambda = float(lambdaD);
      } else if (doLineSearch) {
        const double scaledError = 1e-3 * curError;
        double gd = 0.0;
        if (doLineSearch == 2) {
          double part = 0.0;
          for (int c = tid; c < n; c += 256) {
            part += m.g[c] * m.x[c];
          }
          gd = blockSumD(s.red, part, tid);
        }
        float scale = 1.f;
        for (int ls = 0; ls < 10; ++ls) {
          for (int i = tid; i < P; i += 256) {
            m.Y[i] = m.th[i];
          }
          __syncthreads();
          for (int c = tid; c < n; c += 256) {
            m.Y[fv.solveList[c]] -= double(scale) * m.x[c];
          }
          __syncthreads();
          const double eNew = blockErrorD<true>(rv, pb, s, m, m.Y, b, U, tid, mixLevel, &stateError, mixRecP, &rig, hasParamRows);
          if ((curError - eNew) >= (doLineSearch == 2 ? double(1e-4f * scale) * gd : double(scale) * scaledError)) {
            break;
          }
          scale *= 0.5f;
        }
        for (int i = tid; i < P; i += 256) {
          m.th[i] = m.Y[i];
        }
        stateValid = !hasParamRows;
      } else {
        for (int c = tid; c < n; c += 256) {
          m.th[fv.solveList[c]] -= m.x[c];
        }
        stateValid = false;
      }
      break;
    }
    if (kTR) {
      if (trNoStep) {
        break;
      }
      for (int i = tid; i < P; i += 256) {
        s.dfull[i] = s.th[i];
      }
      __syncthreads();
      for (int c = tid; c < n; c += 256) {
        s.dfull[fv.solveList[c]] -= s.d0[c];
      }
      __syncthreads();
      const double eNew = blockError<kGen, false, !kCsrLds>(rig, rv, pb, fv, s, s.dfull, b, tid);
      const float predicted = trDg + (trMu - 1e-20f) * trDn2;
      const float rho = float((curError - eNew) / double(predicted));
      if (rho < 0.25f) {
        trRadius = 0.25f * trRadius;
      } else if (rho > 0.75f) {
        trRadius = fminf(2.f * trRadius, 10.f);
      }
      if (rho > 0.f) {
        for (int i = tid; i < P; i += 256) {
          s.th[i] = s.dfull[i];
        }
        break;
      }
      if (++trustStep >= 10) {
        break;
      }
      __syncthreads();
      continue;
    }
    if (!notPd && stepRule == 1) {
      float part = 0.f;
      for (int c = tid; c < n; c += 256) {
        part += s.d0[c] * s.g[c] + lambda * s.d0[c] * s.d0[c];
      }
      const float predicted = blockSumF(s, part, tid);
      for (int i = tid; i < P; i += 256) {
        s.dfull[i] = s.th[i];
      }
      __syncthreads();
      for (int c = tid; c < n; c += 256) {
        s.dfull[fv.solveList[c]] -= s.d0[c];
      }
      __syncthreads();
      double eFull = 0.0;
      const double eNew = blockError<kGen, kReuse, !kCsrLds>(rig, rv, pb, fv, s, s.dfull, b, tid, &eFull);
      const float rho = predicted > 0.f ? float((curError - eNew) / double(predicted)) : -1.f;
      if (st.stepHistory != nullptr && tid == 0) {
        double* sh = st.stepHistory + (size_t(b) * fp.maxIterations + it) * 2;
        sh[0] = double(lambda);
        sh[1] = double(rho);
      }
      stateValid = false;
      if (rho > 0.f) {
        for (int i = tid; i < P; i += 256) {
          s.th[i] = s.dfull[i];
        }
        stateValid = kReuse && !hasParamRows;
        stateError = eFull;
      }
      if (!(rho >= 0.25f)) {
        lambda = fminf(lambda * fp.lmUp, fp.lmLambdaMax);
      } else if (rho > 0.75f) {
        lambda = fmaxf(lambda * fp.lmDown, fp.lmLambdaMin);
      }
    } else if (notPd && stepRule == 1) {
      if (st.stepHistory != nullptr && tid == 0) {
        double* sh = st.stepHistory + (size_t(b) * fp.maxIterations + it) * 2;
        sh[0] = double(lambda);
        sh[1] = -1.0;
      }
      lambda = fminf(lambda * fp.lmUp, fp.lmLambdaMax);
    } else if (!notPd && doLineSearch) {
      const float scaledError = 1e-3f * float(curError);
      double gd = 0.0;
      if (doLineSearch == 2) {
        float part = 0.f;
        for (int c = tid; c < n; c += 256) {
          part += s.g[c] * s.d0[c];
        }
        gd = double(blockSumF(s, part, tid));
      }
      float scale = 1.f;
      for (int ls = 0; ls < 10; ++ls) {
        for (int i = tid; i < P; i += 256) {
          s.dfull[i] = s.th[i];
        }
        __syncthreads();
        for (int c = tid; c < n; c += 256) {
          s.dfull[fv.solveList[c]] -= scale * s.d0[c];
        }
        __syncthreads();
        const double eNew = blockError<kGen, kReuse, !kCsrLds>(rig, rv, pb, fv, s, s.dfull, b, tid, &stateError);
        if ((curError - eNew) >= (doLineSearch == 2 ? double(1e-4f * scale) * gd : double(scale * scaledError))) {
          break;
        }
        scale *= 0.5f;
      }
      for (int i = tid; i < P; i += 256) {
        s.th[i] = s.dfull[i];
      }
      stateValid = kReuse && !hasParamRows;
    } else if (!notPd) {
      for (int c = tid; c < n; c += 256) {
        s.th[fv.solveList[c]] -= s.d0[c];
      }
      stateValid = false;
    }
    break;
    }
    }
    if (st.paramHistory != nullptr) {
      float* ph = st.paramHistory + (size_t(b) * fp.maxIterations + it) * size_t(P);
      for (int i = tid; i < P; i += 256) {
        ph[i] = kMix ? float(m.th[i]) : s.th[i];
      }
    }
    if (wave == 0) {
      float w = pivotWorst;
      w = fmaxf(w, dppMoveF<0xB1>(w));
      w = fmaxf(w, dppMoveF<0x4E>(w));
      w = fmaxf(w, dppMoveF<0x141>(w));
      w = fmaxf(w, dppMoveF<0x140>(w));
      pivotWorst = 0.f;
      if (lane == 0) {
        float e0 = estAcc[2];
        if (e0 < 0.f) {
          e0 = estAcc[2] = float(curError);
        }
        estAcc[0] = fmaxf(estAcc[0], w);
        estAcc[1] = fmaxf(estAcc[1], w * (e0 > 0.f ? sqrtf(float(curError) / e0) : 1.f));
      }
    }
    if (tid == 0) {
      const double e = curError;
      if (st.errorHistory != nullptr) {
        st.errorHistory[size_t(b) * fp.maxIterations + it] = e;
      }
      itersDone = it + 1;
      if (badPivot && !kMix) {
        s.flags[2] |= 2;
      }
      if (floored) {
        s.flags[2] |= 4;
      }

// ... 881 lines not shown
    rhoVec[size_t(b) * NP + c] = a;
  }
}

size_t treeStateFloats(int J, int U) {
  return treeStateLayout(J, U).total;
}
size_t treeRefineLdsBytes(int J, int P, int U, int n, int genRows) {
  return treeRefineLdsFloats(J, P, U, n, nullptr, nullptr, genRows) * sizeof(float);
}

hipError_t launchTreeRefine(
    const RigDev& rig,
    const ProblemDev& pb,
    const FusedDev& fd,
    const float* theta,
    const float* state,
    const float* genState,
    const float* dvec,
    float* rhoVec,
    const int32_t* refState,
    float lambda,
    const float* lambdaPer,
    hipStream_t stream) {
  const size_t lds = treeRefineLdsBytes(rig.layoutJ, rig.P, fd.U, fd.n, fd.genRows);
  if (lds > 160 * 1024 - 64) {
    return hipErrorInvalidValue;
  }
  const bool extra = pb.M > pb.rowsJoint || fd.GT > 0 || pb.instPosParent != nullptr || pb.instOriParent != nullptr;
  if (!extra) {
    constexpr int kRefWaves = 8;
    static LdsLimitCache ldsLimitWide;
    hipError_t rc = ldsLimitWide.ensure(reinterpret_cast<const void*>(treeRefineKernel<kRefWaves>), lds);
    if (rc != hipSuccess) {
      return rc;
    }
    hipLaunchKernelGGL((treeRefineKernel<kRefWaves>), dim3(pb.B), dim3(64 * kRefWaves), lds, stream, rig, pb, fd, theta, state, genState, dvec, rhoVec, refState, lambda, lambdaPer);
    return hipGetLastError();
  }
  static LdsLimitCache ldsLimit;
  {
    hipError_t rc = ldsLimit.ensure(reinterpret_cast<const void*>(treeRefineKernel<4>), lds);
    if (rc != hipSuccess) {
      return rc;
    }
  }
  hipLaunchKernelGGL(treeRefineKernel<4>, dim3(pb.B), dim3(256), lds, stream, rig, pb, fd, theta, state, genState, dvec, rhoVec, refState, lambda, lambdaPer);
  return hipGetLastError();
}
#endif

#if !defined(MMX_FUSED_GROUP) || MMX_FUSED_GROUP == 0
size_t fusedCsrFloats(int J, int nnz) {
  auto a4 = [](size_t x) { return (x + 3) & ~size_t(3); };
  return a4(7 * size_t(J) + 1) + 2 * a4(nnz);
}
size_t fusedLdsBytes(int NB, int J, int P, int U, int nsrc, int n, int numCells, bool cellsBehindRho, int GT, int genRows, bool separateUy, size_t csrFloats, bool mix) {
  return fusedLayout(NB, J, P, U, nsrc, n, numCells, cellsBehindRho, GT, genRows, separateUy, csrFloats, mix).total * sizeof(float);
}
#endif

template <int NB, int MODE, bool kTR, bool kGen = false, int kRule = -1>
static hipError_t launchFusedMode(
    const RigDev& rig,
    const ProblemDev& pb,
    const FusedDev& fd,
    float* theta,
    const SolveStateDev& st,
    const FusedParams& fp,
    float* dbgH,
    float* dbgG,
    long long* dbgClk,
    void* argsBuf,
    hipStream_t stream) {
  constexpr bool kFourL = FusedFour<NB, kTR, kGen, kRule>::value;
  const size_t lds = fusedLdsBytes(NB, rig.layoutJ, rig.P, fd.U, fd.nsrc, fd.n, fd.numCells, kRule < 0, kGen ? fd.GT : 0, kGen ? fd.genRows : 0, kTR, kFourL ? 0 : fusedCsrFloats(rig.layoutJ, fd.nnz));
  if (lds > 160 * 1024) {
    return hipErrorInvalidValue;
  }
  constexpr bool kLazyBuilt = kFourL && MODE == 0;
  const bool lazy = kLazyBuilt && argsBuf != nullptr && rig.instPreRot == nullptr && rig.instOffset == nullptr && pb.fnWeights == nullptr;
  if (lazy) {
    static LdsLimitCache ldsLimit;
    hipError_t rc = ldsLimit.ensure(reinterpret_cast<const void*>(fusedSolveKernel<NB, MODE, kTR, kGen, kRule, kLazyBuilt>), lds);
    if (rc != hipSuccess) {
      return rc;
    }
    FusedArgs* dst = static_cast<FusedArgs*>(argsBuf);
    hipLaunchKernelGGL(stashFusedArgsKernel, dim3(1), dim3(1), 0, stream, FusedArgs{rig, pb, fd, st, fp}, dst);
    hipLaunchKernelGGL((fusedSolveKernel<NB, MODE, kTR, kGen, kRule, kLazyBuilt>), dim3(pb.B), dim3(256), lds, stream, dst, RigDev{}, ProblemDev{}, FusedDev{}, theta, SolveStateDev{}, FusedParams{}, dbgH, dbgG, dbgClk, MixSelect{});
  } else {
    static LdsLimitCache ldsLimit;
    hipError_t rc = ldsLimit.ensure(reinterpret_cast<const void*>(fusedSolveKernel<NB, MODE, kTR, kGen, kRule, false>), lds);
    if (rc != hipSuccess) {
      return rc;
    }
    hipLaunchKernelGGL((fusedSolveKernel<NB, MODE, kTR, kGen, kRule, false>), dim3(pb.B), dim3(256), lds, stream, static_cast<const FusedArgs*>(nullptr), rig, pb, fd, theta, st, fp, dbgH, dbgG, dbgClk, MixSelect{});
  }
  return hipGetLastError();
}

template <int NB>
static hipError_t launchFusedNB(
    const RigDev& rig,
    const ProblemDev& pb,
    const FusedDev& fd,
    float* theta,
    const SolveStateDev& st,
    const FusedParams& fp,
    float* dbgH,
    float* dbgG,
    long long* dbgClk,
    void* argsBuf,
    hipStream_t stream) {
  if (fd.GT > 0) {
    if (fp.stepRule == 2) {
      return hipErrorInvalidValue;
    }
    if (dbgH != nullptr || dbgG != nullptr) {
      return launchFusedMode<NB, 1, false, true>(rig, pb, fd, theta, st, fp, dbgH, dbgG, nullptr, argsBuf, stream);
    }
    return launchFusedMode<NB, 0, false, true>(rig, pb, fd, theta, st, fp, nullptr, nullptr, nullptr, argsBuf, stream);
  }
  if (fp.stepRule == 2) {
    return launchFusedMode<NB, 0, true>(rig, pb, fd, theta, st, fp, nullptr, nullptr, nullptr, argsBuf, stream);
  }
  if (dbgClk != nullptr) {
    return launchFusedMode<NB, 2, false>(rig, pb, fd, theta, st, fp, dbgH, dbgG, dbgClk, argsBuf, stream);
  }
  if (dbgH != nullptr || dbgG != nullptr) {
    return launchFusedMode<NB, 1, false>(rig, pb, fd, theta, st, fp, dbgH, dbgG, dbgClk, argsBuf, stream);
  }
  if (pb.M == pb.rowsJoint) {
    if (fp.stepRule == 0 && fp.doLineSearch == 0) {
      return launchFusedMode<NB, 0, false, false, 0>(rig, pb, fd, theta, st, fp, nullptr, nullptr, nullptr, argsBuf, stream);
    }
    if (fp.stepRule == 1) {
      return launchFusedMode<NB, 0, false, false, 1>(rig, pb, fd, theta, st, fp, nullptr, nullptr, nullptr, argsBuf, stream);
    }
  }
  return launchFusedMode<NB, 0, false>(rig, pb, fd, theta, st, fp, dbgH, dbgG, dbgClk, argsBuf, stream);
}

template <int NB>
static hipError_t launchFusedMixedNB(const RigDev& rig, const ProblemDev& pb, const FusedDev& fd, float* theta, const SolveStateDev& st, const FusedParams& fp, const MixSelect& sel, int blocks, long long* dbgClk, hipStream_t stream) {
  const size_t lds = fusedLdsBytes(NB, rig.layoutJ, rig.P, fd.U, fd.nsrc, fd.n, fd.numCells, true, 0, 0, false, 0, true);
  if (lds > 160 * 1024) {
    return hipErrorInvalidValue;
  }
  if (NB == 6 && dbgClk != nullptr) {
// ... 54 lines not shown
#elif MMX_FUSED_GROUP == 2
hipError_t launchFusedGroup2(int nb, MMX_FUSED_ARGS) {
  switch (nb) {
    MMX_CASE(7) MMX_CASE(8) MMX_CASE(10) default : return hipErrorInvalidValue;
  }
}
#elif MMX_FUSED_GROUP == 9
#ifndef MMX_PROBE_RULE
#define MMX_PROBE_RULE 0
#endif
template __global__ void fusedSolveKernel<6, 0, false, false, MMX_PROBE_RULE, true>(
    const FusedArgs*, RigDev, ProblemDev, FusedDev, float*, SolveStateDev, FusedParams, float*, float*, long long*, MixSelect);
#elif MMX_FUSED_GROUP == 8
template __global__ void fusedSolveKernel<6, 0, false, false, -1, false, true>(
    const FusedArgs*, RigDev, ProblemDev, FusedDev, float*, SolveStateDev, FusedParams, float*, float*, long long*, MixSelect);
#elif MMX_FUSED_GROUP == 3
hipError_t launchFusedGroup3(int nb, MMX_FUSED_ARGS) {
  switch (nb) {
    MMX_CASE(12) MMX_CASE(14) default : return hipErrorInvalidValue;
  }
}
#elif MMX_FUSED_GROUP == 5
hipError_t launchFusedMixedGroup5(int nb, MMX_MIXED_ARGS) {
  switch (nb) {
    MMX_MIXED_CASE(1) MMX_MIXED_CASE(2) MMX_MIXED_CASE(3) MMX_MIXED_CASE(4) default : return hipErrorInvalidValue;
  }
}
#elif MMX_FUSED_GROUP == 6
hipError_t launchFusedMixedGroup6(int nb, MMX_MIXED_ARGS) {
  switch (nb) {
    MMX_MIXED_CASE(5) MMX_MIXED_CASE(6) MMX_MIXED_CASE(7) MMX_MIXED_CASE(8) default : return hipErrorInvalidValue;
  }
}
#endif
#undef MMX_CASE
#undef MMX_MIXED_CASE

#if MMX_FUSED_GROUP == 0
int fusedBlocksFor(int n) {
  const int nb = (n + 15) / 16;
  const int avail[] = {1, 2, 3, 4, 5, 6, 7, 8, 10, 12, 14};
  for (int a : avail) {
    if (nb <= a) {
      return a;
    }
  }
  return -1;
}

size_t fusedArgsBytes() {
  return sizeof(FusedArgs);
}

bool fusedMixedUsable(int J, int P, int U, int nsrc, int n, int numCells) {
  const int nb = fusedBlocksFor(n);
  return nb >= 1 && nb <= 8 && J <= 256 && fusedLdsBytes(nb, J, P, U, nsrc, n, numCells, true, 0, 0, false, 0, true) <= 160 * 1024;
}
hipError_t launchFusedMixed(MMX_MIXED_ARGS) {
  const int nb = fusedBlocksFor(fd.n);
  if (nb < 1 || nb > 8) {
    return hipErrorInvalidValue;
  }
  return nb <= 4 ? launchFusedMixedGroup5(nb, rig, pb, fd, theta, st, fp, sel, blocks, dbgClk, stream) : launchFusedMixedGroup6(nb, rig, pb, fd, theta, st, fp, sel, blocks, dbgClk, stream);
}

hipError_t launchFusedSolve(MMX_FUSED_ARGS) {
  const int nb = fusedBlocksFor(fd.n);
  if (nb < 0) {
    return hipErrorInvalidValue;
  }
  if (nb <= 3) {
    return launchFusedGroup0(nb, MMX_FUSED_PASS);
  }
  if (nb <= 6) {
    return launchFusedGroup1(nb, MMX_FUSED_PASS);
  }
  if (nb <= 10) {
    return launchFusedGroup2(nb, MMX_FUSED_PASS);
  }
  return launchFusedGroup3(nb, MMX_FUSED_PASS);
}
#endif

}
```

### momentum_amd/csrc/mmx_fused_helpers.hpp

```cpp
#pragma once

#include "mmx_device.hpp"
#include "mmx_kernels.hpp"
#include "mmx_tree.hpp"

namespace mmx {

struct FusedLds {
  int16_t* mStart;
  int* mTin;
  int* mInfo;
  float* mW;
  float* th;
  float* js;
  float* up;
  float* ur;
  float* uy;
  float* us;
  float* own1;
  float* sub1;
  float* g;
  float* d0;
  float* rho;
  float* invDiag;
  float* dfull;
  float* jd;
  float* tanOwn;
  float* tanPre;
  double* red;
  int* flags;
  float* gEv;
  float* gRes;
  float* gW;
  float* gJ;
  double* fkA;
  double* fkB;
  float* own2;
  float* umom;
  float* sub2;
  float* L;
  float* srcT;
};

struct RigView {
  int32_t J, P, R, numLevels, jumpRounds;
  const int32_t* parent;
  const float* preRot;
  const float* offset;
  const int32_t* ptOuter;
  const int32_t* ptInner;
  const float* ptValue;
  const float* ptOffsets;
  bool hasOffsets;
  const int32_t* levelOrder;
  const int32_t* levelStart;
  const int4* rowRec;
  int32_t numRowRec;
};
template <class I>
struct FusedViewT {
  int32_t U, Kp;
  const I* subSize;
  const I* dfsJoint;
  const I* loadedPos;
  int32_t numLoaded;
  const I* colToSolve;
  const I* unitPos;
  const I* posUnitStart;
  const I* posUnits;
  const I* solveList;
};
using FusedView = FusedViewT<int32_t>;
using FusedViewS = FusedViewT<int16_t>;

__host__ __device__ __forceinline__ size_t alignUp4(size_t x) {
  return (x + 3) & ~size_t(3);
}
__host__ __device__ __forceinline__ int srcStrideFor(int nsrc) {
  int x = (nsrc + 15) & ~15;
  return (x & 31) == 16 ? x : x + 16;
}
constexpr int kSrcCh = 15;

__device__ __forceinline__ void firstOrderMoments(float* o, F3 p, float yx, float yy, float yz, bool point) {
  o[3] = p.y * yz - p.z * yy;
  o[4] = p.z * yx - p.x * yz;
  o[5] = p.x * yy - p.y * yx;
  o[0] = point ? yx : 0.f;
  o[1] = point ? yy : 0.f;
  o[2] = point ? yz : 0.f;
  o[6] = point ? p.x * yx + p.y * yy + p.z * yz : 0.f;
}

template <int NCH, int STRIDE, int kT = 256, class FV = FusedView, bool kSecondOnly = false>
__device__ __forceinline__ void gatherOwnSums(const FV& fd, const FusedLds& s, const float* umom, int tid) {
  for (int item = tid; item < fd.numLoaded * NCH; item += kT) {
    const int li = item / NCH, c = item - li * NCH;
    const int k = fd.loadedPos[li];
    float acc = 0.f;
    const int e1 = fd.posUnitStart[k + 1];
    for (int e = fd.posUnitStart[k]; e < e1; ++e) {
      acc += umom[STRIDE * fd.posUnits[e] + c];
    }
    if (kSecondOnly) {
      s.own2[kC2 * k + c] = acc;
    } else if (c < kC1) {
      s.own1[kC1 * k + c] = acc;
    } else {
      s.own2[kC2 * k + (c - kC1)] = acc;
    }
  }
}
constexpr int kUmom = 25;

template <int kT = 256, class FV = FusedView, bool kSecondOnly = false>
__device__ __forceinline__ void ownSums(const FV& fd, const FusedLds& s, float* umom, int U, int tid, const double* upD = nullptr, const double* usD = nullptr) {
  constexpr int NCH = kSecondOnly ? kC2Used : kC1 + kC2Used;
  for (int u = tid; u < U; u += kT) {
    const F3 p = kSecondOnly ? F3{float(upD[3 * u]), float(upD[3 * u + 1]), float(upD[3 * u + 2])} : F3{s.up[3 * u], s.up[3 * u + 1], s.up[3 * u + 2]};
    const bool point = u < fd.Kp;
    float* o = umom + kUmom * u;
    if (!kSecondOnly) {
      firstOrderMoments(o, p, s.uy[3 * u], s.uy[3 * u + 1], s.uy[3 * u + 2], point);
    }
    const float sg = kSecondOnly ? float(usD[u]) : s.us[u];
    const float s2 = sg * sg;
    float* o2 = kSecondOnly ? o : o + kC1;
#pragma unroll
    for (int c = 0; c < kC2Used; ++c) {
      o2[c] = 0.f;
    }
    const int q = point ? 4 : 10;
    o2[q + 0] = s2 * p.x * p.x;
    o2[q + 1] = s2 * p.x * p.y;
    o2[q + 2] = s2 * p.x * p.z;
    o2[q + 3] = s2 * p.y * p.y;
    o2[q + 4] = s2 * p.y * p.z;
    o2[q + 5] = s2 * p.z * p.z;
    if (point) {
      o2[0] = s2;
      o2[1] = s2 * p.x;
      o2[2] = s2 * p.y;
      o2[3] = s2 * p.z;
    }
  }
  __syncthreads();
  gatherOwnSums<NCH, kUmom, kT, FV, kSecondOnly>(fd, s, umom, tid);
}

constexpr int kFusedTreeUn = 4;
template <int NC, bool kSubtree, int STRIDE = NC, int UN = kFusedTreeUn, class I = int32_t>
__device__ __forceinline__ void treeSum(const FusedViewT<I>& fd, const float* in, float* out, int J, int wave, int lane, const int32_t* kRange = nullptr) {
  treeSumT<NC, kSubtree, STRIDE, UN, I>(fd.subSize, fd.loadedPos, fd.numLoaded, in, out, J, wave, 4, lane, kRange);
}

struct ParamCol {
  float g, h;
};

template <class I = int32_t>
__device__ __forceinline__ ParamCol paramRowsColumn(
    const RigDev& rig,
    const ProblemDev& pb,
    const FusedDev& fd,
    const float* th,
    const float* d0,
// ... 83 lines not shown
    }
  }
  if (pb.hasModel && pb.wModel > 0.f) {
    const float* tp = pb.mpTarget + size_t(b) * P;
    const float* tw = pb.mpWeights + size_t(b) * P;
    double em = 0.0;
    for (int i = tid; i < P; i += 256) {
      if (pb.enabledMask[i] != 0) {
        const double w = double(tw[i]);
        if (!kJacobianRows || w > 0.0) {
          const double pd = w * (th[i] - double(tp[i]));
          em += pd * pd;
        }
      }
    }
    e += em * double(pb.wModel) * 1e-1;
  }
  return e;
}

template <int kT = 256, typename Gather, typename Store>
__device__ __forceinline__ void csrRowsPrefetched(const int32_t* outer, const int32_t* inner, const float* value, int R, int tid, Gather x, Store out) {
  for (int r0 = tid; r0 < R; r0 += 4 * kT) {
    int ka[4], kb[4], in0[4];
    float v0[4];
#pragma unroll
    for (int i = 0; i < 4; ++i) {
      const int r = min(r0 + kT * i, R - 1);
      ka[i] = outer[r], kb[i] = outer[r + 1];
    }
#pragma unroll
    for (int i = 0; i < 4; ++i) {
      const bool has = kb[i] > ka[i];
      in0[i] = has ? inner[ka[i]] : 0, v0[i] = has ? value[ka[i]] : 0.f;
    }
#pragma unroll
    for (int i = 0; i < 4; ++i) {
      const int r = r0 + kT * i;
      if (r < R) {
        decltype(x(0)) acc = 0;
        if (kb[i] > ka[i]) {
          acc += v0[i] * x(in0[i]);
          for (int k = ka[i] + 1; k < kb[i]; ++k) {
            acc += value[k] * x(inner[k]);
          }
        }
        out(r, acc);
      }
    }
  }
}

template <int kT = 256, typename Gather, typename Store>
__device__ __forceinline__ void csrRowsFromRecords(const int4* rec, int numRec, const int32_t* inner, const float* value, int R, int tid, Gather x, Store out) {
  for (int t = tid; t < numRec; t += kT) {
    const int4 q = rec[t];
    const int row = q.x & 0xffff, span = int(uint32_t(q.x) >> 16), in0 = q.y & 0xffff, cnt = int(uint32_t(q.y) >> 16);
    auto acc = __int_as_float(q.z) * x(in0);
    for (int k = q.w + 1; k < q.w + cnt; ++k) {
      acc += value[k] * x(inner[k]);
    }
    out(row, acc);
    for (int r = row + 1; r < row + span; ++r) {
      out(r, decltype(acc)(0));
    }
    if (t == 0) {
      for (int r = 0; r < row; ++r) {
        out(r, decltype(acc)(0));
      }
    }
  }
}

template <bool kGlobalTables = false, int kT = 256>
__device__ __forceinline__ void
blockFk(const RigView& rig, const FusedLds& s, const float* th, int tid, bool withAxes, long long* clk = nullptr, long long* clkLast = nullptr) {
  auto stamp = [&](int slot) {
    if (clk != nullptr && blockIdx.x == 0 && threadIdx.x == 0) {
      const long long now = clock64();
      clk[slot] += now - *clkLast;
      *clkLast = now;
    }
  };
  if (kGlobalTables && rig.rowRec != nullptr) {
    csrRowsFromRecords<kT>(
        rig.rowRec, rig.numRowRec, rig.ptInner, rig.ptValue, rig.R, tid, [&](int c) { return th[c]; }, [&](int r, float acc) { s.jd[r] = acc + (rig.hasOffsets ? rig.ptOffsets[r] : 0.f); });
  } else if (kGlobalTables) {
    csrRowsPrefetched<kT>(
        rig.ptOuter, rig.ptInner, rig.ptValue, rig.R, tid, [&](int c) { return th[c]; }, [&](int r, float acc) { s.jd[r] = acc + (rig.hasOffsets ? rig.ptOffsets[r] : 0.f); });
  } else {
    for (int r = tid; r < rig.R; r += kT) {
      const float off = rig.hasOffsets ? rig.ptOffsets[r] : 0.f;
      float acc = 0.f;
      const int k1 = rig.ptOuter[r + 1];
      for (int k = rig.ptOuter[r]; k < k1; ++k) {
        acc += rig.ptValue[k] * th[rig.ptInner[k]];
      }
      s.jd[r] = acc + off;
    }
  }
  float pre[4] = {0.f, 0.f, 0.f, 1.f}, off3[3] = {0.f, 0.f, 0.f};
  if (tid < rig.J) {
#pragma unroll
    for (int d = 0; d < 4; ++d) {
      pre[d] = rig.preRot[4 * tid + d];
    }
#pragma unroll
    for (int d = 0; d < 3; ++d) {
      off3[d] = rig.offset[3 * tid + d];
    }
  }
  __syncthreads();
  stamp(26);
  const int Jp = fkPad(rig.J);
  for (int j = tid; j < rig.J; j += kT) {
    float* slot = s.js + kJs * j;
    float loc[8];
    if (j == tid) {
      fkLocalFromParams(s.jd + 7 * j, pre, off3, loc, slot + 8);
    } else {
      fkLocalFromParams(s.jd + 7 * j, rig.preRot + 4 * j, rig.offset + 3 * j, loc, slot + 8);
    }
    if (rig.jumpRounds == 0) {
#pragma unroll
      for (int c = 0; c < 8; ++c) {
        slot[c] = loc[c];
      }
    } else {
      fkStoreLocalD(s.fkA, Jp, j, loc, rig.parent[j] + 1);
    }
  }
  __syncthreads();
  stamp(24);
  fkJumpRoundsD(s.js, s.fkA, s.fkB, rig.J, rig.jumpRounds, tid, kT);
  stamp(25);
  if (withAxes) {
    for (int j = tid; j < rig.J; j += kT) {
// ... 8 lines not shown
```

### momentum_amd/csrc/mmx_kernels.hpp

```cpp
#pragma once

#include <atomic>

#include <hip/hip_runtime.h>

#include <cstddef>
#include <cstdint>

#include "mmx_device.hpp"

namespace mmx {

struct SolveStateDev {
  int32_t* done;
  int32_t* iterations;
  int32_t* status;
  double* lastError;
  double* finalError;
  double* errorHistory;
  float* paramHistory;
  double* stepHistory;
  float* diag;
  float precisionBound;
};
// ... 43 lines not shown
struct StepParams {
  float lambda;
  float threshold;
  int32_t iteration;
  int32_t minIterations;
  int32_t maxIterations;
  int32_t refine;
  float* delta;
  int32_t* stepIter;
  float* lambdaPer;
  double* stepHistory;
  float* diagErr0;
  float* diagAcc;
  TrustStateDev tr;
  int32_t doLineSearch;
  int32_t stepRule;
  float lmLambdaMin, lmLambdaMax, lmUp, lmDown;
  long long* clk;
  const uint32_t* tileMasks;
  int32_t numTiles;
};

struct FusedDev {
  int32_t U, Kp, n, nsrc, nnz;
  int32_t slotBase;
  const int32_t* subSize;
  const int32_t* dfsJoint;
  const int32_t* loadedPos;
  int32_t numLoaded;
  const int32_t* unitJoint;
  const int32_t* posUnitStart;
  const int32_t* posUnits;
  const int32_t* solveList;
  const int32_t* srcStart;
  const ColumnSourceDev* srcs;
  const uint4* gTerms;
  int32_t termRounds;
  const uint4* gTerms16;
  int32_t termRounds16;
  const int32_t* comb;
  int32_t numComb;
  int32_t numCells;
  int32_t numLimits;
  const int32_t* limStart;
  const int32_t* limOf;
  int32_t numPairDests;
  const int32_t* pairDest;
  const int32_t* pairCols;
  const int32_t* pairStart;
  const int32_t* pairLim;
  int32_t GT, genRows;
  const int32_t* tileList;
  int32_t numTiles;
};

struct FusedParams {
  float lambda;
  float threshold;
  int32_t minIterations;
  int32_t maxIterations;
  int32_t refine;
  int32_t doLineSearch;
  int32_t stepRule;
  float lmLambdaMin, lmLambdaMax, lmUp, lmDown;
  float trustRadius;
  float mixTol;
  int32_t mixMaxCg;
  int32_t autoAbort;
};

struct MixSelect {
  const int32_t* map;
  const int32_t* count;
  const float* thetaInit;
};

size_t fusedLdsBytes(int NB, int J, int P, int U, int nsrc, int n, int numCells, bool cellsBehindRho, int GT = 0, int genRows = 0, bool separateUy = false, size_t csrFloats = 0, bool mix = false);
size_t fusedCsrFloats(int J, int nnz);
size_t treeNormalEquationsLdsBytes(int J, int P, int U, int nsrc, int n, int GT = 0, int genRows = 0);
size_t treeRefineLdsBytes(int J, int P, int U, int n, int genRows);
size_t treeGenStateFloats(int n, int genRows);
hipError_t launchTreeNormalEquations(
    const RigDev& rig,
    const ProblemDev& pb,
    const FusedDev& fd,
    const float* theta,
    float* jtj,
    float* jtr,
    const int32_t* done,
    double* errOut,
    float* state,
    long long* clk,
    float* genState,
    bool tileMajor,
    hipStream_t stream);
size_t treeStateFloats(int J, int U);
hipError_t launchTreeRefine(
    const RigDev& rig,
    const ProblemDev& pb,
    const FusedDev& fd,
    const float* theta,
    const float* state,
    const float* genState,
    const float* dvec,
    float* rhoVec,
    const int32_t* refState,
    float lambda,
    const float* lambdaPer,
    hipStream_t stream);
size_t gradientLdsBytes(int J, int P, int U);
hipError_t launchEvalGradient(const RigDev& rig, const ProblemDev& pb, const FusedDev& fd, const float* theta, float* grad, double* err, hipStream_t stream);
int fusedBlocksFor(int n);
hipError_t launchFusedSolve(
    const RigDev& rig,
    const ProblemDev& pb,
    const FusedDev& fd,
    float* theta,
    const SolveStateDev& st,
    const FusedParams& fp,
    float* dbgH,
    float* dbgG,
    long long* dbgClk,
    void* argsBuf,
    hipStream_t stream);
size_t fusedArgsBytes();
bool fusedMixedUsable(int J, int P, int U, int nsrc, int n, int numCells);
hipError_t launchFusedMixed(
    const RigDev& rig, const ProblemDev& pb, const FusedDev& fd, float* theta, const SolveStateDev& st, const FusedParams& fp, const MixSelect& sel, int blocks, long long* dbgClk, hipStream_t stream);

size_t waveLdsBytes(int J, int P, int U, int n, bool frames = false);
// ... 125 lines not shown
```

### momentum_amd/csrc/mmx_mixed.hpp

```cpp
#pragma once

#include "mmx_device.hpp"
#include "mmx_device_d.hpp"

namespace mmx {

constexpr int kJsD = 17;
constexpr int kTanD = 8;
constexpr float kMixFactorDamping = 1e-6f;
constexpr double kLn2D = 0.693147180559945309417232121458176568;

struct MixLds {
  double* th;
  double* js;
  double* up;
  double* uf;
  double* us;
  double* g;
  double* x;
  double* r;
  double* p;
  double* q;
  double* X;
  double* Y;
  int16_t* lo;
  int16_t* hi;
  int layoutJ;
};
__host__ __device__ inline size_t mixXDoubles(int J, int nsrc) {
  return size_t(7 * J > nsrc ? 7 * J : nsrc);
}
__host__ __device__ inline size_t mixYDoubles(int J, int P) {
  return size_t(kTanD * J > P ? kTanD * J : P);
}
__host__ __device__ inline size_t mixPersistentDoubles(int J, int P, int U, int NP) {
  return size_t(P) + size_t(kJsD) * J + 7 * size_t(U) + 5 * size_t(NP);
}

__device__ __forceinline__ void mixSinCos(double x, double* sOut, double* cOut) {
  if (!(fabs(x) < 1e5)) {
    x = fma(-rint(x * 1.59154943091895335769e-01), 6.28318530717958647693e+00, x);
  }
  const double fn = rint(x * 6.36619772367581382433e-01);
  double r = fma(-fn, 1.57079632673412561417e+00, x);
  r = fma(-fn, 6.07710050650619224932e-11, r);
  const int q = int(fn) & 3;
  const double z = r * r;
  const double ps = 8.33333333332248946124e-03 + z * (-1.98412698298579493134e-04 + z * (2.75573137070700676789e-06 + z * (-2.50507602534068634195e-08 + z * 1.58969099521155010221e-10)));
  const double sn = r + (z * r) * (-1.66666666666666324348e-01 + z * ps);
  const double pc = z * (4.16666666666666019037e-02 + z * (-1.38888888888741095749e-03 + z * (2.48015872894767294178e-05 + z * (-2.75573143513906633035e-07 + z * (2.08757232129817482790e-09 + z * -1.13596475577881948265e-11)))));
  const double hz = 0.5 * z, w = 1.0 - hz;
  const double cs = w + (((1.0 - w) - hz) + z * pc);
  const double sv = (q & 1) ? cs : sn, cv = (q & 1) ? sn : cs;
  *sOut = (q & 2) ? -sv : sv;
  *cOut = ((q + 1) & 2) ? -cv : cv;
}
__device__ __forceinline__ void fkLocalFromParamsD(const double* p, const float* pre, const float* off, double* o, double* oq) {
  double sx, cx, sy, cy, sz, cz;
  mixSinCos(0.5 * p[3], &sx, &cx);
  mixSinCos(0.5 * p[4], &sy, &cy);
  mixSinCos(0.5 * p[5], &sz, &cz);
  const DQ q0{double(pre[0]), double(pre[1]), double(pre[2]), double(pre[3])};
  const DQ q1 = dqmul(q0, DQ{0.0, 0.0, sz, cz});
  const DQ q2 = dqmul(q1, DQ{0.0, sy, 0.0, cy});
  const DQ ql = dqmul(q2, DQ{sx, 0.0, 0.0, cx});
  o[0] = double(off[0]) + p[0], o[1] = double(off[1]) + p[1], o[2] = double(off[2]) + p[2];
  o[3] = ql.x, o[4] = ql.y, o[5] = ql.z, o[6] = ql.w;
  o[7] = exp2(p[6]);
  oq[0] = q1.x, oq[1] = q1.y, oq[2] = q1.z, oq[3] = q1.w;
  oq[4] = q2.x, oq[5] = q2.y, oq[6] = q2.z, oq[7] = q2.w;
}
__device__ __forceinline__ void fkStoreLocalDD(double* bufA, int Jp, int j, const double* o, int parentPlus1) {
  FkXf x;
  x.tx = o[0], x.ty = o[1], x.tz = o[2], x.qx = o[3], x.qy = o[4], x.qz = o[5], x.qw = o[6];
  x.s = o[7], x.jl = parentPlus1;
  fkStoreD(bufA, Jp, j, x);
}
__device__ __forceinline__ void fkAxesInPlaceD(const float* pre, int j, int par, double* js) {
  DQ qp{0.0, 0.0, 0.0, 1.0};
  if (par >= 0) {
    const double* p = js + kJsD * par;
    qp = DQ{p[3], p[4], p[5], p[6]};
  }
  double* o = js + kJsD * j;
  const D3 az = dqrot(dqmul(qp, DQ{double(pre[0]), double(pre[1]), double(pre[2]), double(pre[3])}), D3{0.0, 0.0, 1.0});
  const D3 ay = dqrot(dqmul(qp, DQ{o[8], o[9], o[10], o[11]}), D3{0.0, 1.0, 0.0});
  const D3 ax = dqrot(dqmul(qp, DQ{o[12], o[13], o[14], o[15]}), D3{1.0, 0.0, 0.0});
  o[8] = ax.x, o[9] = ax.y, o[10] = ax.z;
  o[11] = ay.x, o[12] = ay.y, o[13] = ay.z;
  o[14] = az.x, o[15] = az.y, o[16] = az.z;
// ... 106 lines not shown
```

### momentum_amd/csrc/mmx_tree.hpp

```cpp
#pragma once

#include "mmx_device.hpp"

namespace mmx {

__device__ __forceinline__ F3 transAxisCol(const float* js, int parent, int d) {
  if (parent < 0) {
    return F3{d == 0 ? 1.f : 0.f, d == 1 ? 1.f : 0.f, d == 2 ? 1.f : 0.f};
  }
  const float* p = js + kJs * parent;
  const F3 c = qmatCol(Q4{p[3], p[4], p[5], p[6]}, d);
  return F3{c.x * p[7], c.y * p[7], c.z * p[7]};
}

constexpr int kC2 = 17;
constexpr int kC2Used = 16;
constexpr int kC1 = 7;

template <int NC, bool kSubtree, int STRIDE = NC, int UN = 1, class I = int32_t>
__device__ __forceinline__ void treeSumT(
    const I* subSize,
    const I* loadedPos,
    int numLoaded,
    const float* in,
    float* out,
    int J,
    int wave,
    int numWaves,
    int lane,
    const int32_t* kRange = nullptr) {
  const int K = kSubtree ? numLoaded : J;
  const int rowTiles = (J + 15) >> 4;
  constexpr int colTiles = (NC + 15) / 16;
  const int i = lane & 15, g = lane >> 4;
  for (int t = wave; t < rowTiles * colTiles; t += numWaves) {
    const int rt = t / colTiles, ct = t - rt * colTiles;
    const int r = 16 * rt + i;
    const int rsz = r < J ? subSize[r] : 0;
    const int c = 16 * ct + i;
    v4f acc{0.f, 0.f, 0.f, 0.f};
    const int kEnd = kSubtree ? (kRange != nullptr ? kRange[2 * rt + 1] : K) : (K < 16 * rt + 16 ? K : 16 * rt + 16);
    const int kBegin = kSubtree && kRange != nullptr ? kRange[2 * rt] : 0;
    for (int k0 = kBegin; k0 < kEnd; k0 += 4 * UN) {
      int pp[UN], sz[UN];
      float bv[UN];
#pragma unroll
      for (int u = 0; u < UN; ++u) {
        const int kk = k0 + 4 * u + g;
        pp[u] = kSubtree ? loadedPos[kk < kEnd ? kk : 0] : kk;
      }
#pragma unroll
      for (int u = 0; u < UN; ++u) {
        const int kk = k0 + 4 * u + g;
        sz[u] = kSubtree ? 0 : subSize[kk < kEnd ? pp[u] : 0];
        bv[u] = (kk < kEnd && c < NC) ? in[STRIDE * pp[u] + c] : 0.f;
      }
#pragma unroll
      for (int u = 0; u < UN; ++u) {
        const int kk = k0 + 4 * u + g, p = pp[u];
        const bool m = kSubtree ? (p >= r && p < r + rsz) : (r < J && p <= r && r < p + sz[u]);
        acc = __builtin_amdgcn_mfma_f32_16x16x4f32((kk < kEnd && m) ? 1.f : 0.f, bv[u], acc, 0, 0, 0);
      }
    }
#pragma unroll
    for (int q = 0; q < 4; ++q) {
      const int orow = 16 * rt + 4 * g + q, ocol = 16 * ct + i;
      if (orow < J && ocol < NC) {
        out[STRIDE * orow + ocol] = acc[q];
      }
    }
// ... 45 lines not shown
```

Before: 2.245 million solves/s.

## Keep constraint payloads and CSR row records resident in LDS for fused solve

Adds a resident-inputs mode, on by default, to the fused solve kernel. Each workgroup copies its per-unit constraint payloads and the parameter-transform CSR row records and entries into spare LDS once, then reads them from LDS on every Gauss-Newton iteration and line-search error evaluation instead of from global memory. Joint tables are also sized to the live joint count to free LDS. Each piece is only placed if it fits the per-CU LDS budget, so occupancy is kept, but the change adds a one-time fill cost and more layout complexity.

```diff
diff --git a/include/mmx.h b/include/mmx.h
--- a/include/mmx.h
+++ b/include/mmx.h
@@ -212,11 +212,13 @@
   float mixed_tolerance;
   int32_t mixed_max_cg;
   int32_t joint_pruning;
-  int32_t reserved[3];
+  int32_t resident_inputs;
+  int32_t reserved[2];
 } mmx_tuning;
 int32_t mmx_problem_set_tuning(mmx_problem* problem, const mmx_tuning* tuning);
 int32_t mmx_problem_last_route(const mmx_problem* problem);
 int32_t mmx_problem_num_solve_joints(const mmx_problem* problem);
+int32_t mmx_problem_resident_inputs(const mmx_problem* problem);
 
 int32_t mmx_problem_num_rows(const mmx_problem* problem);
 int32_t mmx_problem_batch(const mmx_problem* problem);
diff --git a/momentum_amd/_abi.py b/momentum_amd/_abi.py
--- a/momentum_amd/_abi.py
+++ b/momentum_amd/_abi.py
@@ -325,7 +325,7 @@
 
 class Tuning(C.Structure):
 
-    _fields_ = [("route", C.c_int32), ("max_refinement_steps", C.c_int32), ("mixed_tolerance", C.c_float), ("mixed_max_cg", C.c_int32), ("joint_pruning", C.c_int32), ("reserved", C.c_int32 * 3)]
+    _fields_ = [("route", C.c_int32), ("max_refinement_steps", C.c_int32), ("mixed_tolerance", C.c_float), ("mixed_max_cg", C.c_int32), ("joint_pruning", C.c_int32), ("resident_inputs", C.c_int32), ("reserved", C.c_int32 * 2)]
 
 
 def as_ptr(a: np.ndarray, ctype):
diff --git a/momentum_amd/build.py b/momentum_amd/build.py
--- a/momentum_amd/build.py
+++ b/momentum_amd/build.py
@@ -58,7 +58,7 @@
     except (OSError, ValueError):
         return {}
 SOURCE_DEPS = {"mmx_wave_frames.hip": ["mmx_wave.hip"]}
-HEADERS = ["mmx_device.hpp", "mmx_device_d.hpp", "mmx_kernels.hpp", "mmx_tree.hpp", "mmx_fused_helpers.hpp", "mmx_host_tables.hpp", "mmx_solve_plan.hpp", "mmx_constraint_intake.hpp", os.path.join("..", "..", "include", "mmx.h")]
+HEADERS = ["mmx_device.hpp", "mmx_device_d.hpp", "mmx_kernels.hpp", "mmx_tree.hpp", "mmx_fused_helpers.hpp", "mmx_fused_layout.hpp", "mmx_mixed.hpp", "mmx_host_tables.hpp", "mmx_solve_plan.hpp", "mmx_constraint_intake.hpp", os.path.join("..", "..", "include", "mmx.h")]
 ARCH = "gfx950"
 
 
diff --git a/momentum_amd/capi.py b/momentum_amd/capi.py
--- a/momentum_amd/capi.py
+++ b/momentum_amd/capi.py
@@ -18,7 +18,7 @@
     "mmx_gn_options_default", "mmx_abi_version", "mmx_last_error", "mmx_device_count",
     "mmx_rig_create", "mmx_rig_destroy", "mmx_rig_num_joints", "mmx_rig_num_params",
     "mmx_problem_create", "mmx_problem_destroy", "mmx_problem_num_rows", "mmx_problem_batch",
-    "mmx_problem_set_tuning", "mmx_problem_last_route", "mmx_problem_num_solve_joints",
+    "mmx_problem_set_tuning", "mmx_problem_last_route", "mmx_problem_num_solve_joints", "mmx_problem_resident_inputs",
     "mmx_problem_set_enabled", "mmx_problem_set_constraints", "mmx_problem_set_constraints_sized", "mmx_problem_set_instance_rig", "mmx_problem_set_instance_parents", "mmx_eval_jacobian", "mmx_eval_jacobian_timed", "mmx_debug_store_pattern",
     "mmx_eval_skeleton_state", "mmx_eval_normal_equations", "mmx_solve", "mmx_solve_with_history", "mmx_solve_with_step_history", "mmx_problem_solve_diagnostics", "mmx_solve_f64", "mmx_solve_f64_host", "mmx_solve_host",
     "mmx_solve_frames", "mmx_solve_frames_host",
@@ -66,6 +66,8 @@
     L.mmx_problem_set_tuning.argtypes = [vp, C.POINTER(_abi.Tuning)]
     L.mmx_problem_last_route.argtypes = [vp]
     L.mmx_problem_num_solve_joints.argtypes = [vp]
+    L.mmx_problem_resident_inputs.restype = C.c_int32
+    L.mmx_problem_resident_inputs.argtypes = [vp]
     L.mmx_problem_set_constraints.argtypes = [vp, C.POINTER(ConstraintData), vp]
     L.mmx_problem_set_constraints_sized.argtypes = [vp, C.POINTER(ConstraintData), C.c_size_t, vp]
     L.mmx_problem_set_instance_rig.argtypes = [vp, vp, vp, i32, vp]
@@ -289,6 +291,7 @@
         t.max_refinement_steps = int(max_refinement_steps)
         t.mixed_tolerance, t.mixed_max_cg = getattr(self, "_mixed", (0.0, 0))
         t.joint_pruning = 0 if getattr(self, "_joint_pruning", True) else -1
+        t.resident_inputs = 0 if getattr(self, "_resident_inputs", True) else -1
         self._route_args = (route, int(max_refinement_steps))
         _check(lib().mmx_problem_set_tuning(self._h, C.byref(t)))
 
@@ -299,6 +302,13 @@
     def set_joint_pruning(self, on: bool = True) -> None:
         self._joint_pruning = bool(on)
         self._set_tuning(*getattr(self, "_route_args", ("auto", 0)))
+
+    def set_resident_inputs(self, on: bool = True) -> None:
+        self._resident_inputs = bool(on)
+        self._set_tuning(*getattr(self, "_route_args", ("auto", 0)))
+
+    def resident_inputs(self) -> int:
+        return int(lib().mmx_problem_resident_inputs(self._h))
 
     def num_solve_joints(self) -> int:
         return int(lib().mmx_problem_num_solve_joints(self._h))
diff --git a/momentum_amd/csrc/mmx_capi.hip b/momentum_amd/csrc/mmx_capi.hip
--- a/momentum_amd/csrc/mmx_capi.hip
+++ b/momentum_amd/csrc/mmx_capi.hip
@@ -536,6 +536,7 @@
 }
 SolveView solveView(const mmx_problem* pb) {
   SolveView v{pb->rigDev, pb->dev, pb->fdev};
+  v.fd.residentInputs = pb->tuning.resident_inputs == 0 ? 1 : 0;
   if (!solveViewActive(pb)) {
     return v;
   }
@@ -1052,6 +1053,9 @@
   }
   if (tuning->joint_pruning != 0 && tuning->joint_pruning != -1) {
     return fail(MMX_ERR_INVALID_ARGUMENT, "mmx_tuning::joint_pruning: 0 (on) or -1 (off)");
+  }
+  if (tuning->resident_inputs != 0 && tuning->resident_inputs != -1) {
+    return fail(MMX_ERR_INVALID_ARGUMENT, "mmx_tuning::resident_inputs: 0 (on) or -1 (off)");
   }
   for (int32_t r : tuning->reserved) {
     if (r != 0) {
@@ -2043,6 +2047,20 @@
 }
 }
 
+int32_t mmx_problem_resident_inputs(const mmx_problem* pb) {
+  if (pb == nullptr || pb->rig == nullptr || pb->tuning.resident_inputs != 0) {
+    return 0;
+  }
+  mmx_gn_options o;
+  mmx_gn_options_default(&o);
+  const mmx::SolvePlan plan = mmx::planSolve(solveFacts(pb, SolveOutputs{}, MMX_PRECISION_F32, pb->tuning.route == MMX_ROUTE_WAVE), o);
+  if (plan.code != MMX_OK || plan.numStages < 1 || plan.stages[0].kind != mmx::SolveStageKind::Single || plan.stages[0].route != MMX_ROUTE_FUSED) {
+    return 0;
+  }
+  const SolveView sv = solveView(pb);
+  return mmx::fusedResidentInputs(sv.rig, sv.pb, sv.fd);
+}
+
 int32_t mmx_solve(
     mmx_problem* pb,
     const mmx_gn_options* o,
diff --git a/momentum_amd/csrc/mmx_device.hpp b/momentum_amd/csrc/mmx_device.hpp
--- a/momentum_amd/csrc/mmx_device.hpp
+++ b/momentum_amd/csrc/mmx_device.hpp
@@ -6,10 +6,10 @@
 
 #include "../../include/mmx.h"
 #include "mmx_constraint_intake.hpp"
+#include "mmx_fused_layout.hpp"
 
 namespace mmx {
 
-constexpr int kJs = 17;
 constexpr float kPivotFloor = 3.814697265625e-6f;
 constexpr float kFactorDamping = 1e-5f;
 constexpr float kPrecisionGain = 0.042f;
@@ -290,13 +290,6 @@
   fkLocalSplit(rig, j, theta, o, o + 8);
 }
 
-constexpr int kFkCh = 9;
-__host__ __device__ __forceinline__ int fkPad(int J) {
-  return (J + 1) & ~1;
-}
-__host__ __device__ __forceinline__ size_t fkBufFloats(int J) {
-  return 2 * size_t(kFkCh) * size_t(fkPad(J));
-}
 struct FkXf {
   double tx, ty, tz, qx, qy, qz, qw, s;
   int jl;
@@ -963,7 +956,6 @@
 
 typedef float v4f __attribute__((ext_vector_type(4)));
 
-constexpr int kTan = 9;
 
 __device__ __forceinline__ int tileAddr(int row, int col) {
   return row * 16 + ((((col >> 2) ^ (row >> 2)) & 3) << 2) + (col & 3);
diff --git a/momentum_amd/csrc/mmx_fused.hip b/momentum_amd/csrc/mmx_fused.hip
--- a/momentum_amd/csrc/mmx_fused.hip
+++ b/momentum_amd/csrc/mmx_fused.hip
@@ -272,51 +272,26 @@
   __syncthreads();
 }
 
-constexpr int kGenEv = 29;
-
 template <int NB, bool kTR, bool kGen, int kRule>
 struct FusedFour {
   static constexpr bool value = NB <= 6 && !kGen && !kTR;
 };
 
-struct FusedLayout {
-  size_t uyFloats;
-  size_t auxOff;
-  size_t cellOff;
-  size_t t9;
-  size_t arenaFloats;
-  size_t umomFloats;
-  size_t regionFloats;
-  size_t genFloats;
-  size_t total;
-};
-__host__ __device__ inline FusedLayout fusedLayout(int NB, int J, int P, int U, int nsrc, int n, int numCells, bool cellsBehindRho, int GT, int genRows, bool separateUy = false, size_t csrFloats = 0, bool mix = false) {
-  auto a4 = [](size_t x) { return (x + 3) & ~size_t(3); };
-  auto h4 = [&](size_t x) { return a4((x + 1) / 2); };
-  auto mx = [](size_t x, size_t y) { return x > y ? x : y; };
-  const size_t T = size_t(NB) * (NB + 1) / 2, NP = 16 * size_t(NB);
-  FusedLayout l;
-  l.cellOff = cellsBehindRho ? 2 * NP : 0;
-  const size_t aux = a4(mx(2 * NP, mx(size_t(nsrc), l.cellOff + size_t(numCells))));
-  l.auxOff = separateUy ? a4(3 * size_t(U)) : 0;
-  l.uyFloats = separateUy ? l.auxOff + aux : mx(a4(3 * size_t(U)), aux);
-  l.t9 = a4(size_t(kTan) * J);
-  l.arenaFloats = mx(size_t(kSrcCh - 1) * size_t(srcStrideFor(nsrc)), 2 * l.t9 + a4(P));
-  if (mix) {
-    l.arenaFloats = mx(size_t(kSrcCh - 1) * size_t(srcStrideFor(nsrc)), a4(2 * (mixXDoubles(J, nsrc) + mixYDoubles(J, P))));
-  }
-  l.umomFloats = mx(a4(size_t(kUmom) * U), a4(size_t(kC1) * J));
-  const size_t scratch = fkBufFloats(J) + 2 * a4(size_t(kC2) * J) + l.umomFloats;
-  l.regionFloats = mx(scratch, T * 256);
-  const size_t rowsGp = a4(size_t(genRows));
-  l.genFloats = GT > 0 ? a4(size_t(kGenEv) * GT) + 2 * a4(rowsGp) + a4(rowsGp * size_t(srcStrideFor(int(NP)))) : 0;
-  const size_t meta = h4(NP + 1) + 3 * a4(nsrc) + a4(J) + 4 * h4(J) + h4(size_t(J) + 1) + 2 * h4(U) + h4(n) + h4(P);
-  size_t fixed = a4(P) + a4(size_t(kJs) * J) + 2 * a4(3 * size_t(U)) + a4(U) + 2 * a4(NP) + l.uyFloats + 16 + 8;
-  if (mix) {
-    fixed = l.uyFloats + 40 + 8 + a4(2 * mixPersistentDoubles(J, P, U, int(NP))) + 2 * h4(J);
-  }
-  l.total = meta + fixed + l.genFloats + l.arenaFloats + l.regionFloats + csrFloats;
-  return l;
+__host__ __device__ inline FusedShape fusedShapeFor(int NB, bool kTR, bool kGen, int kRule, bool kMix, const RigDev& rig, const FusedDev& fd, size_t csrFloats) {
+  FusedShape s;
+  s.NB = NB, s.layoutJ = rig.layoutJ, s.liveJ = rig.J, s.P = rig.P, s.U = fd.U, s.Kp = fd.Kp, s.nsrc = fd.nsrc, s.n = fd.n;
+  s.numCells = fd.numCells, s.cellsBehindRho = kRule < 0;
+  s.GT = kGen ? fd.GT : 0, s.genRows = kGen ? fd.genRows : 0;
+  s.separateUy = kTR, s.csrFloats = csrFloats, s.mix = kMix;
+  s.numRowRec = rig.ptRowRec != nullptr ? rig.numRowRec : 0;
+  s.nnz = fd.nnz;
+  s.perCu = fusedWorkgroupsPerCu(NB, kTR, kGen, kMix);
+  s.resident = !kMix && fd.residentInputs != 0;
+  return s;
+}
+template <int NB, bool kTR, bool kGen, int kRule, bool kMix>
+__host__ __device__ inline FusedShape fusedShapeOf(const RigDev& rig, const FusedDev& fd, size_t csrFloats) {
+  return fusedShapeFor(NB, kTR, kGen, kRule, kMix, rig, fd, csrFloats);
 }
 
 __device__ __forceinline__ double generalRowsError(const ProblemDev& pb, const float* js, int b, int tid) {
@@ -461,7 +436,7 @@
   }
 }
 
-template <bool kGen = false, bool kStore = false, bool kGlobalCsr = true, class FV = FusedViewS>
+template <bool kGen = false, bool kStore = false, bool kGlobalCsr = true, class FV = FusedViewS, bool kResident = false>
 __device__ __forceinline__ double blockError(
     const RigDev& rigDev,
     const RigView& rig,
@@ -473,10 +448,11 @@
     int tid,
     double* unrounded = nullptr) {
   const int lane = tid & 63, wave = tid >> 6;
-  blockFk<kGlobalCsr>(rig, s, th, tid, kStore);
+  blockFk<kGlobalCsr, 256, kResident>(rig, s, th, tid, kStore);
   double e = 0.0;
+  const float* resPay = kResident ? residentPayload(s) : nullptr;
   for (int u = tid; u < fd.U; u += 256) {
-    const Unit un = evalUnit(pb, s.js, b, u);
+    const Unit un = resPay != nullptr ? evalUnitFrom(pb, residentUnitInput(resPay, fd, u), s.js, u) : evalUnit(pb, s.js, b, u);
     if (kStore) {
       s.up[3 * u] = un.v.x, s.up[3 * u + 1] = un.v.y, s.up[3 * u + 2] = un.v.z;
       const float rx = un.sigma * un.f.x, ry = un.sigma * un.f.y, rz = un.sigma * un.f.z;
@@ -964,7 +940,8 @@
   constexpr bool kLeanOps = kFour;
   constexpr bool kLeanAcc = kFour;
   const int kNnz = fd.nnz;
-  const FusedLayout lay = fusedLayout(NB, JL, P, U, nsrc, n, fd.numCells, kRule < 0, kGen ? fd.GT : 0, kGen ? fd.genRows : 0, kTR, 0, kMix);
+  const FusedLayout lay = fusedLayout(fusedShapeOf<NB, kTR, kGen, kRule, kMix>(rig, fd, kCsrLds ? fusedCsrFloatsFor(JL, kNnz) : 0));
+  const int JT = lay.tableJ;
   MixLds m{};
   m.layoutJ = JL;
   {
@@ -979,15 +956,15 @@
     s.mTin = reinterpret_cast<int*>(take(nsrc));
     s.mInfo = reinterpret_cast<int*>(take(nsrc));
     s.mW = take(nsrc);
-    lParent = reinterpret_cast<int*>(take(JL));
-    lParentPos = takeS(JL);
-    lSubSize = takeS(JL);
-    lPosUnitStart = takeS(JL + 1);
+    lParent = reinterpret_cast<int*>(take(JT));
+    lParentPos = takeS(JT);
+    lSubSize = takeS(JT);
+    lPosUnitStart = takeS(JT + 1);
     lPosUnits = takeS(U);
     lUnitJoint = takeS(U);
     lSolveList = takeS(n);
-    lDfsJoint = takeS(JL);
-    lLoadedPos = takeS(JL);
+    lDfsJoint = takeS(JT);
+    lLoadedPos = takeS(JT);
     lColToSolve = takeS(P);
     if (kCsrLds) {
       lPtOuter = reinterpret_cast<int*>(take(kR + 1));
@@ -1000,7 +977,7 @@
       m.hi = takeS(JL);
     } else {
       s.th = take(P);
-      s.js = take(size_t(kJs) * JL);
+      s.js = take(size_t(kJs) * JT);
       s.up = take(3 * size_t(U));
       s.ur = take(3 * size_t(U));
       s.us = take(U);
@@ -1049,6 +1026,10 @@
     }
   }
 
+  float* const resPay0 = !kMix && lay.payloadFloats > 0 ? smem + lay.payloadOff : nullptr;
+  int4* const resRec0 = !kMix && lay.rowRecWords > 0 ? reinterpret_cast<int4*>(smem + lay.rowRecOff) : nullptr;
+  int2* const resEnt0 = !kMix && lay.rowEntWords > 0 ? reinterpret_cast<int2*>(smem + lay.rowEntOff) : nullptr;
+
   float* thg = theta + size_t(b) * P;
   if (kMix) {
     const float* th0 = sel.thetaInit != nullptr ? sel.thetaInit + size_t(b) * P : thg;
@@ -1147,6 +1128,9 @@
     s.flags[0] = 0;
     s.flags[1] = 0;
     s.flags[2] = 0;
+    const float* fl = reinterpret_cast<const float*>(s.flags);
+    s.flags[7] = int(uint32_t(resPay0 != nullptr ? (resPay0 - fl) >> 2 : 0) | (uint32_t(resRec0 != nullptr ? (reinterpret_cast<const float*>(resRec0) - fl) >> 2 : 0) << 14) |
+                     (resEnt0 != nullptr ? 1u << 28 : 0u));
     estAcc[0] = estAcc[1] = 0.f, estAcc[2] = -1.f;
   }
   int4 mixRec{0, 0, 0, 0};
@@ -1155,6 +1139,27 @@
     mixRec = rv.rowRec[tid];
   }
   const MixRowRec mixRecP{mixRec, mixHasRec};
+  if (resPay0 != nullptr) {
+    for (int u = tid; u < U; u += 256) {
+      if (u < fd.Kp || (u - fd.Kp) % 3 == 0) {
+        storeUnitPayload(resPay0, loadUnitInput(pb, b, u), fd.Kp, u);
+      }
+    }
+  }
+  if (resRec0 != nullptr) {
+    for (int t = tid; t < rv.numRowRec; t += 256) {
+      resRec0[t] = rv.rowRec[t];
+    }
+  }
+  if (resEnt0 != nullptr) {
+    for (int t = tid; t < rv.numRowRec; t += 256) {
+      const int4 q = rv.rowRec[t];
+      const int cnt = int(uint32_t(q.y) >> 16);
+      for (int k = q.w + 1; k < q.w + cnt; ++k) {
+        resEnt0[k - t - 1] = int2{rv.ptInner[k], __float_as_int(rv.ptValue[k])};
+      }
+    }
+  }
   int mixLevel = 0;
   if (kMix && tid < J) {
     for (int a = lParent[tid]; a >= 0; a = lParent[a]) {
@@ -1201,7 +1206,7 @@
     const int lane = tid & 63;
     const int wave = __builtin_amdgcn_readfirstlane(tid >> 6);
     constexpr bool kLateUnit = kFour || kMix;
-    const UnitInput uin0 = kLateUnit ? UnitInput{} : loadUnitInput(pb, b, tid < U ? tid : U);
+    const UnitInput uin0 = (kLateUnit || (!kMix && lay.payloadFloats > 0)) ? UnitInput{} : loadUnitInput(pb, b, tid < U ? tid : U);
     float trLambda = 1e-10f;
     int trustStep = 0;
     bool trNoStep = false;
@@ -1234,12 +1239,13 @@
       curError = (s.red[0] + s.red[1]) + (s.red[2] + s.red[3]);
       MMX_CLK(1)
     } else {
-    blockFk<!kCsrLds>(rv, s, s.th, tid, true, MODE == 2 ? dbgClk : nullptr, &clkLast);
+    blockFk<!kCsrLds, 256, true>(rv, s, s.th, tid, true, MODE == 2 ? dbgClk : nullptr, &clkLast);
     MMX_CLK(1)
     {
       double e = 0.0;
+      const float* resPay = residentPayload(s);
       for (int u = tid; u < U; u += 256) {
-        const Unit un = evalUnitFrom(pb, (!kLateUnit && u == tid) ? uin0 : loadUnitInput(pb, b, u), s.js, u);
+        const Unit un = evalUnitFrom(pb, resPay != nullptr ? residentUnitInput(resPay, fv, u) : ((!kLateUnit && u == tid) ? uin0 : loadUnitInput(pb, b, u)), s.js, u);
         s.up[3 * u] = un.v.x, s.up[3 * u + 1] = un.v.y, s.up[3 * u + 2] = un.v.z;
         const float rx = un.sigma * un.f.x, ry = un.sigma * un.f.y, rz = un.sigma * un.f.z;
         s.ur[3 * u] = rx, s.ur[3 * u + 1] = ry, s.ur[3 * u + 2] = rz;
@@ -1896,6 +1902,8 @@
             }
             od(r, a);
           }
+        } else if (const int4* recLds = residentRowRecords(s)) {
+          csrRowsFromRecords<256>(recLds, rv.numRowRec, rv.ptInner, rv.ptValue, rv.R, tid, xd, od, residentRowEntries(s, rv.numRowRec));
         } else if (rv.rowRec != nullptr) {
           csrRowsFromRecords<256>(rv.rowRec, rv.numRowRec, rv.ptInner, rv.ptValue, rv.R, tid, xd, od);
         } else {
@@ -2234,7 +2242,7 @@
         s.dfull[fv.solveList[c]] -= s.d0[c];
       }
       __syncthreads();
-      const double eNew = blockError<kGen, false, !kCsrLds>(rig, rv, pb, fv, s, s.dfull, b, tid);
+      const double eNew = blockError<kGen, false, !kCsrLds, FusedViewS, true>(rig, rv, pb, fv, s, s.dfull, b, tid);
       const float predicted = trDg + (trMu - 1e-20f) * trDn2;
       const float rho = float((curError - eNew) / double(predicted));
       if (rho < 0.25f) {
@@ -2269,7 +2277,7 @@
       }
       __syncthreads();
       double eFull = 0.0;
-      const double eNew = blockError<kGen, kReuse, !kCsrLds>(rig, rv, pb, fv, s, s.dfull, b, tid, &eFull);
+      const double eNew = blockError<kGen, kReuse, !kCsrLds, FusedViewS, true>(rig, rv, pb, fv, s, s.dfull, b, tid, &eFull);
       const float rho = predicted > 0.f ? float((curError - eNew) / double(predicted)) : -1.f;
       if (st.stepHistory != nullptr && tid == 0) {
         double* sh = st.stepHistory + (size_t(b) * fp.maxIterations + it) * 2;
@@ -2316,7 +2324,7 @@
           s.dfull[fv.solveList[c]] -= scale * s.d0[c];
         }
         __syncthreads();
-        const double eNew = blockError<kGen, kReuse, !kCsrLds>(rig, rv, pb, fv, s, s.dfull, b, tid, &stateError);
+        const double eNew = blockError<kGen, kReuse, !kCsrLds, FusedViewS, true>(rig, rv, pb, fv, s, s.dfull, b, tid, &stateError);
         if ((curError - eNew) >= (doLineSearch == 2 ? double(1e-4f * scale) * gd : double(scale * scaledError))) {
           break;
         }
@@ -3304,13 +3312,17 @@
 
 #if !defined(MMX_FUSED_GROUP) || MMX_FUSED_GROUP == 0
 size_t fusedCsrFloats(int J, int nnz) {
-  auto a4 = [](size_t x) { return (x + 3) & ~size_t(3); };
-  return a4(7 * size_t(J) + 1) + 2 * a4(nnz);
+  return fusedCsrFloatsFor(J, nnz);
 }
 size_t fusedLdsBytes(int NB, int J, int P, int U, int nsrc, int n, int numCells, bool cellsBehindRho, int GT, int genRows, bool separateUy, size_t csrFloats, bool mix) {
-  return fusedLayout(NB, J, P, U, nsrc, n, numCells, cellsBehindRho, GT, genRows, separateUy, csrFloats, mix).total * sizeof(float);
+  return fusedLayoutPlain(NB, J, P, U, nsrc, n, numCells, cellsBehindRho, GT, genRows, separateUy, csrFloats, mix).total * sizeof(float);
 }
 #endif
+
+static bool staticLdsWithin(const void* kernel) {
+  hipFuncAttributes a{};
+  return hipFuncGetAttributes(&a, kernel) == hipSuccess && a.sharedSizeBytes <= kFusedStaticLdsBytes;
+}
 
 template <int NB, int MODE, bool kTR, bool kGen = false, int kRule = -1>
 static hipError_t launchFusedMode(
@@ -3326,28 +3338,33 @@
     void* argsBuf,
     hipStream_t stream) {
   constexpr bool kFourL = FusedFour<NB, kTR, kGen, kRule>::value;
-  const size_t lds = fusedLdsBytes(NB, rig.layoutJ, rig.P, fd.U, fd.nsrc, fd.n, fd.numCells, kRule < 0, kGen ? fd.GT : 0, kGen ? fd.genRows : 0, kTR, kFourL ? 0 : fusedCsrFloats(rig.layoutJ, fd.nnz));
+  constexpr bool kLazyBuilt = kFourL && MODE == 0;
+  const bool lazy = kLazyBuilt && argsBuf != nullptr && rig.instPreRot == nullptr && rig.instOffset == nullptr && pb.fnWeights == nullptr;
+  const void* kernel = lazy ? reinterpret_cast<const void*>(fusedSolveKernel<NB, MODE, kTR, kGen, kRule, kLazyBuilt>)
+                            : reinterpret_cast<const void*>(fusedSolveKernel<NB, MODE, kTR, kGen, kRule, false>);
+  FusedDev fdL = fd;
+  if (fdL.residentInputs != 0) {
+    static const bool fitsLazy = staticLdsWithin(reinterpret_cast<const void*>(fusedSolveKernel<NB, MODE, kTR, kGen, kRule, kLazyBuilt>));
+    static const bool fitsPlain = staticLdsWithin(reinterpret_cast<const void*>(fusedSolveKernel<NB, MODE, kTR, kGen, kRule, false>));
+    if (!(lazy ? fitsLazy : fitsPlain)) {
+      fdL.residentInputs = 0;
+    }
+  }
+  const size_t lds = fusedLayout(fusedShapeOf<NB, kTR, kGen, kRule, false>(rig, fdL, kFourL ? 0 : fusedCsrFloatsFor(rig.layoutJ, fdL.nnz))).total * sizeof(float);
   if (lds > 160 * 1024) {
     return hipErrorInvalidValue;
   }
-  constexpr bool kLazyBuilt = kFourL && MODE == 0;
-  const bool lazy = kLazyBuilt && argsBuf != nullptr && rig.instPreRot == nullptr && rig.instOffset == nullptr && pb.fnWeights == nullptr;
+  static LdsLimitCache ldsLimitLazy, ldsLimitPlain;
+  hipError_t rc = (lazy ? ldsLimitLazy : ldsLimitPlain).ensure(kernel, lds);
+  if (rc != hipSuccess) {
+    return rc;
+  }
   if (lazy) {
-    static LdsLimitCache ldsLimit;
-    hipError_t rc = ldsLimit.ensure(reinterpret_cast<const void*>(fusedSolveKernel<NB, MODE, kTR, kGen, kRule, kLazyBuilt>), lds);
-    if (rc != hipSuccess) {
-      return rc;
-    }
     FusedArgs* dst = static_cast<FusedArgs*>(argsBuf);
-    hipLaunchKernelGGL(stashFusedArgsKernel, dim3(1), dim3(1), 0, stream, FusedArgs{rig, pb, fd, st, fp}, dst);
+    hipLaunchKernelGGL(stashFusedArgsKernel, dim3(1), dim3(1), 0, stream, FusedArgs{rig, pb, fdL, st, fp}, dst);
     hipLaunchKernelGGL((fusedSolveKernel<NB, MODE, kTR, kGen, kRule, kLazyBuilt>), dim3(pb.B), dim3(256), lds, stream, dst, RigDev{}, ProblemDev{}, FusedDev{}, theta, SolveStateDev{}, FusedParams{}, dbgH, dbgG, dbgClk, MixSelect{});
   } else {
-    static LdsLimitCache ldsLimit;
-    hipError_t rc = ldsLimit.ensure(reinterpret_cast<const void*>(fusedSolveKernel<NB, MODE, kTR, kGen, kRule, false>), lds);
-    if (rc != hipSuccess) {
-      return rc;
-    }
-    hipLaunchKernelGGL((fusedSolveKernel<NB, MODE, kTR, kGen, kRule, false>), dim3(pb.B), dim3(256), lds, stream, static_cast<const FusedArgs*>(nullptr), rig, pb, fd, theta, st, fp, dbgH, dbgG, dbgClk, MixSelect{});
+    hipLaunchKernelGGL((fusedSolveKernel<NB, MODE, kTR, kGen, kRule, false>), dim3(pb.B), dim3(256), lds, stream, static_cast<const FusedArgs*>(nullptr), rig, pb, fdL, theta, st, fp, dbgH, dbgG, dbgClk, MixSelect{});
   }
   return hipGetLastError();
 }
@@ -3508,6 +3525,17 @@
   return sizeof(FusedArgs);
 }
 
+int fusedResidentInputs(const RigDev& rig, const ProblemDev& pb, const FusedDev& fd) {
+  const int nb = fusedBlocksFor(fd.n);
+  if (nb < 0) {
+    return 0;
+  }
+  const bool gen = fd.GT > 0;
+  const int rule = !gen && pb.M == pb.rowsJoint ? 0 : -1;
+  const bool four = fusedFourPerCu(nb, false, gen, false);
+  return fusedResidentMask(fusedLayout(fusedShapeFor(nb, false, gen, rule, false, rig, fd, four ? 0 : fusedCsrFloatsFor(rig.layoutJ, fd.nnz))));
+}
+
 bool fusedMixedUsable(int J, int P, int U, int nsrc, int n, int numCells) {
   const int nb = fusedBlocksFor(n);
   return nb >= 1 && nb <= 8 && J <= 256 && fusedLdsBytes(nb, J, P, U, nsrc, n, numCells, true, 0, 0, false, 0, true) <= 160 * 1024;
diff --git a/momentum_amd/csrc/mmx_fused_helpers.hpp b/momentum_amd/csrc/mmx_fused_helpers.hpp
--- a/momentum_amd/csrc/mmx_fused_helpers.hpp
+++ b/momentum_amd/csrc/mmx_fused_helpers.hpp
@@ -73,14 +73,6 @@
 using FusedView = FusedViewT<int32_t>;
 using FusedViewS = FusedViewT<int16_t>;
 
-__host__ __device__ __forceinline__ size_t alignUp4(size_t x) {
-  return (x + 3) & ~size_t(3);
-}
-__host__ __device__ __forceinline__ int srcStrideFor(int nsrc) {
-  int x = (nsrc + 15) & ~15;
-  return (x & 31) == 16 ? x : x + 16;
-}
-constexpr int kSrcCh = 15;
 
 __device__ __forceinline__ void firstOrderMoments(float* o, F3 p, float yx, float yy, float yz, bool point) {
   o[3] = p.y * yz - p.z * yy;
@@ -111,7 +103,6 @@
     }
   }
 }
-constexpr int kUmom = 25;
 
 template <int kT = 256, class FV = FusedView, bool kSecondOnly = false>
 __device__ __forceinline__ void ownSums(const FV& fd, const FusedLds& s, float* umom, int U, int tid, const double* upD = nullptr, const double* usD = nullptr) {
@@ -301,13 +292,20 @@
 }
 
 template <int kT = 256, typename Gather, typename Store>
-__device__ __forceinline__ void csrRowsFromRecords(const int4* rec, int numRec, const int32_t* inner, const float* value, int R, int tid, Gather x, Store out) {
+__device__ __forceinline__ void csrRowsFromRecords(const int4* rec, int numRec, const int32_t* inner, const float* value, int R, int tid, Gather x, Store out, const int2* pairs = nullptr) {
   for (int t = tid; t < numRec; t += kT) {
     const int4 q = rec[t];
     const int row = q.x & 0xffff, span = int(uint32_t(q.x) >> 16), in0 = q.y & 0xffff, cnt = int(uint32_t(q.y) >> 16);
     auto acc = __int_as_float(q.z) * x(in0);
-    for (int k = q.w + 1; k < q.w + cnt; ++k) {
-      acc += value[k] * x(inner[k]);
+    if (pairs != nullptr) {
+      for (int k = q.w + 1; k < q.w + cnt; ++k) {
+        const int2 e = pairs[k - t - 1];
+        acc += __int_as_float(e.y) * x(e.x);
+      }
+    } else {
+      for (int k = q.w + 1; k < q.w + cnt; ++k) {
+        acc += value[k] * x(inner[k]);
+      }
     }
     out(row, acc);
     for (int r = row + 1; r < row + span; ++r) {
@@ -321,7 +319,51 @@
   }
 }
 
-template <bool kGlobalTables = false, int kT = 256>
+__device__ __forceinline__ void storeUnitPayload(float* pay, const UnitInput& in, int Kp, int u) {
+  if (u < Kp) {
+    float* w = pay + kPayloadPos * u;
+    w[0] = in.a[0], w[1] = in.a[1], w[2] = in.a[2];
+    w[3] = in.t[0], w[4] = in.t[1], w[5] = in.t[2];
+    w[6] = in.cw;
+  } else if ((u - Kp) % 3 == 0) {
+    float* w = pay + kPayloadPos * Kp + kPayloadOri * ((u - Kp) / 3);
+    w[0] = in.a[0], w[1] = in.a[1], w[2] = in.a[2], w[3] = in.a[3];
+    w[4] = in.t[0], w[5] = in.t[1], w[6] = in.t[2], w[7] = in.t[3];
+    w[8] = in.cw;
+  }
+}
+__device__ __forceinline__ const float* residentPayload(const FusedLds& s) {
+  const uint32_t w = uint32_t(s.flags[7]) & 0x3fffu;
+  return w != 0 ? reinterpret_cast<const float*>(s.flags) + 4 * w : nullptr;
+}
+__device__ __forceinline__ const int4* residentRowRecords(const FusedLds& s) {
+  const uint32_t w = (uint32_t(s.flags[7]) >> 14) & 0x3fffu;
+  return w != 0 ? reinterpret_cast<const int4*>(reinterpret_cast<const float*>(s.flags) + 4 * w) : nullptr;
+}
+__device__ __forceinline__ const int2* residentRowEntries(const FusedLds& s, int numRowRec) {
+  const uint32_t f = uint32_t(s.flags[7]);
+  return (f >> 28) != 0 ? reinterpret_cast<const int2*>(reinterpret_cast<const float*>(s.flags) + 4 * ((f >> 14) & 0x3fffu) + 4 * numRowRec) : nullptr;
+}
+template <class FV>
+__device__ __forceinline__ UnitInput residentUnitInput(const float* pay, const FV& fd, int u) {
+  UnitInput in;
+  in.tin = fd.unitPos[u];
+  in.joint = fd.dfsJoint[in.tin];
+  if (u < fd.Kp) {
+    const float* w = pay + kPayloadPos * u;
+    in.a[0] = w[0], in.a[1] = w[1], in.a[2] = w[2], in.a[3] = 0.f;
+    in.t[0] = w[3], in.t[1] = w[4], in.t[2] = w[5], in.t[3] = 0.f;
+    in.cw = w[6];
+  } else {
+    const float* w = pay + kPayloadPos * fd.Kp + kPayloadOri * ((u - fd.Kp) / 3);
+    in.a[0] = w[0], in.a[1] = w[1], in.a[2] = w[2], in.a[3] = w[3];
+    in.t[0] = w[4], in.t[1] = w[5], in.t[2] = w[6], in.t[3] = w[7];
+    in.cw = w[8];
+  }
+  return in;
+}
+
+template <bool kGlobalTables = false, int kT = 256, bool kResident = false>
 __device__ __forceinline__ void
 blockFk(const RigView& rig, const FusedLds& s, const float* th, int tid, bool withAxes, long long* clk = nullptr, long long* clkLast = nullptr) {
   auto stamp = [&](int slot) {
@@ -331,7 +373,12 @@
       *clkLast = now;
     }
   };
-  if (kGlobalTables && rig.rowRec != nullptr) {
+  const int4* recLds = kGlobalTables && kResident ? residentRowRecords(s) : nullptr;
+  if (recLds != nullptr) {
+    csrRowsFromRecords<kT>(
+        recLds, rig.numRowRec, rig.ptInner, rig.ptValue, rig.R, tid, [&](int c) { return th[c]; }, [&](int r, float acc) { s.jd[r] = acc + (rig.hasOffsets ? rig.ptOffsets[r] : 0.f); },
+        residentRowEntries(s, rig.numRowRec));
+  } else if (kGlobalTables && rig.rowRec != nullptr) {
     csrRowsFromRecords<kT>(
         rig.rowRec, rig.numRowRec, rig.ptInner, rig.ptValue, rig.R, tid, [&](int c) { return th[c]; }, [&](int r, float acc) { s.jd[r] = acc + (rig.hasOffsets ? rig.ptOffsets[r] : 0.f); });
   } else if (kGlobalTables) {
diff --git a/momentum_amd/csrc/mmx_fused_layout.hpp b/momentum_amd/csrc/mmx_fused_layout.hpp
--- /dev/null
+++ b/momentum_amd/csrc/mmx_fused_layout.hpp
@@ -0,0 +1,165 @@
+#pragma once
+
+#include <cstddef>
+#include <cstdint>
+
+#if defined(__HIPCC__)
+#define MMX_HD __host__ __device__
+#else
+#define MMX_HD
+#endif
+
+namespace mmx {
+
+constexpr int kJs = 17;
+constexpr int kFkCh = 9;
+MMX_HD inline int fkPad(int J) {
+  return (J + 1) & ~1;
+}
+MMX_HD inline size_t fkBufFloats(int J) {
+  return 2 * size_t(kFkCh) * size_t(fkPad(J));
+}
+constexpr int kTan = 9;
+constexpr int kC2 = 17;
+constexpr int kC2Used = 16;
+constexpr int kC1 = 7;
+constexpr int kUmom = 25;
+constexpr int kSrcCh = 15;
+constexpr int kGenEv = 29;
+constexpr int kJsD = 17;
+constexpr int kTanD = 8;
+
+MMX_HD inline size_t alignUp4(size_t x) {
+  return (x + 3) & ~size_t(3);
+}
+MMX_HD inline int srcStrideFor(int nsrc) {
+  int x = (nsrc + 15) & ~15;
+  return (x & 31) == 16 ? x : x + 16;
+}
+MMX_HD inline size_t mixXDoubles(int J, int nsrc) {
+  return size_t(7 * J > nsrc ? 7 * J : nsrc);
+}
+MMX_HD inline size_t mixYDoubles(int J, int P) {
+  return size_t(kTanD * J > P ? kTanD * J : P);
+}
+MMX_HD inline size_t mixPersistentDoubles(int J, int P, int U, int NP) {
+  return size_t(P) + size_t(kJsD) * J + 7 * size_t(U) + 5 * size_t(NP);
+}
+
+MMX_HD constexpr bool fusedFourPerCu(int NB, bool kTR, bool kGen, bool kMix) {
+  return NB <= 6 && !kGen && !kTR && !kMix;
+}
+MMX_HD constexpr int fusedWorkgroupsPerCu(int NB, bool kTR, bool kGen, bool kMix) {
+  return NB <= 6 && !kGen ? (fusedFourPerCu(NB, kTR, kGen, kMix) ? 4 : 3) : (NB <= 8 ? 2 : 1);
+}
+constexpr size_t kLdsPerCuBytes = 160 * 1024;
+constexpr size_t kLdsGranuleBytes = 1280;
+constexpr size_t kFusedStaticLdsBytes = 256;
+MMX_HD constexpr size_t fusedLdsBudgetFloats(int perCu) {
+  return ((kLdsPerCuBytes / size_t(perCu)) / kLdsGranuleBytes * kLdsGranuleBytes - kFusedStaticLdsBytes) / sizeof(float);
+}
+
+constexpr int kPayloadPos = 7, kPayloadOri = 9;
+
+struct FusedShape {
+  int NB = 1;
+  int layoutJ = 0;
+  int liveJ = 0;
+  int P = 0, U = 0, Kp = 0, nsrc = 0, n = 0, numCells = 0;
+  bool cellsBehindRho = false;
+  int GT = 0, genRows = 0;
+  bool separateUy = false;
+  size_t csrFloats = 0;
+  bool mix = false;
+  int numRowRec = 0;
+  int nnz = 0;
+  int perCu = 1;
+  bool resident = false;
+};
+
+struct FusedLayout {
+  size_t uyFloats;
+  size_t auxOff;
+  size_t cellOff;
+  size_t t9;
+  size_t arenaFloats;
+  size_t umomFloats;
+  size_t regionFloats;
+  size_t genFloats;
+  int tableJ;
+  size_t payloadOff, payloadFloats;
+  size_t rowRecOff, rowRecWords;
+  size_t rowEntOff, rowEntWords;
+  size_t total;
+};
+MMX_HD inline FusedLayout fusedLayout(const FusedShape& s) {
+  auto a4 = [](size_t x) { return (x + 3) & ~size_t(3); };
+  auto h4 = [&](size_t x) { return a4((x + 1) / 2); };
+  auto mx = [](size_t x, size_t y) { return x > y ? x : y; };
+  const int NB = s.NB, J = s.layoutJ, P = s.P, U = s.U, nsrc = s.nsrc, n = s.n;
+  const bool res = s.resident && !s.mix;
+  const size_t T = size_t(NB) * (NB + 1) / 2, NP = 16 * size_t(NB);
+  FusedLayout l;
+  l.tableJ = res && s.liveJ > 0 && s.liveJ < J ? s.liveJ : J;
+  const size_t JT = size_t(l.tableJ);
+  l.cellOff = s.cellsBehindRho ? 2 * NP : 0;
+  const size_t aux = a4(mx(2 * NP, mx(size_t(nsrc), l.cellOff + size_t(s.numCells))));
+  l.auxOff = s.separateUy ? a4(3 * size_t(U)) : 0;
+  l.uyFloats = s.separateUy ? l.auxOff + aux : mx(a4(3 * size_t(U)), aux);
+  l.t9 = a4(size_t(kTan) * J);
+  l.arenaFloats = mx(size_t(kSrcCh - 1) * size_t(srcStrideFor(nsrc)), 2 * l.t9 + a4(P));
+  if (s.mix) {
+    l.arenaFloats = mx(size_t(kSrcCh - 1) * size_t(srcStrideFor(nsrc)), a4(2 * (mixXDoubles(J, nsrc) + mixYDoubles(J, P))));
+  }
+  l.umomFloats = mx(a4(size_t(kUmom) * U), a4(size_t(kC1) * J));
+  const size_t scratch = fkBufFloats(J) + 2 * a4(size_t(kC2) * J) + l.umomFloats;
+  l.regionFloats = mx(scratch, T * 256);
+  const size_t rowsGp = a4(size_t(s.genRows));
+  l.genFloats = s.GT > 0 ? a4(size_t(kGenEv) * s.GT) + 2 * a4(rowsGp) + a4(rowsGp * size_t(srcStrideFor(int(NP)))) : 0;
+  const size_t meta = h4(NP + 1) + 3 * a4(nsrc) + a4(JT) + 4 * h4(JT) + h4(JT + 1) + 2 * h4(U) + h4(n) + h4(P);
+  size_t fixed = a4(P) + a4(size_t(kJs) * JT) + 2 * a4(3 * size_t(U)) + a4(U) + 2 * a4(NP) + l.uyFloats + 16 + 8;
+  if (s.mix) {
+    fixed = l.uyFloats + 40 + 8 + a4(2 * mixPersistentDoubles(J, P, U, int(NP))) + 2 * h4(J);
+  }
+  l.total = meta + fixed + l.genFloats + l.arenaFloats + l.regionFloats + s.csrFloats;
+  l.payloadOff = l.rowRecOff = l.rowEntOff = l.total;
+  l.payloadFloats = l.rowRecWords = l.rowEntWords = 0;
+  if (res) {
+    const size_t budget = fusedLdsBudgetFloats(s.perCu);
+    const int Ko = (U - s.Kp) / 3;
+    const size_t pay = a4(size_t(kPayloadPos) * size_t(s.Kp) + size_t(kPayloadOri) * size_t(Ko));
+    if (pay > 0 && l.total + pay <= budget) {
+      l.payloadOff = l.total, l.payloadFloats = pay;
+      l.total += pay;
+    }
+    const size_t rec = 4 * size_t(s.numRowRec);
+    l.rowRecOff = l.total;
+    if (rec > 0 && s.csrFloats == 0 && l.total + rec <= budget) {
+      l.rowRecWords = rec;
+      l.total += rec;
+    }
+    const size_t ent = s.nnz > s.numRowRec ? a4(2 * size_t(s.nnz - s.numRowRec)) : 0;
+    l.rowEntOff = l.total;
+    if (l.rowRecWords > 0 && s.nnz > s.numRowRec && l.total + ent <= budget) {
+      l.rowEntWords = ent;
+      l.total += ent;
+    }
+  }
+  return l;
+}
+
+MMX_HD inline size_t fusedCsrFloatsFor(int J, int nnz) {
+  return alignUp4(7 * size_t(J) + 1) + 2 * alignUp4(size_t(nnz));
+}
+MMX_HD inline FusedLayout fusedLayoutPlain(int NB, int J, int P, int U, int nsrc, int n, int numCells, bool cellsBehindRho, int GT, int genRows, bool separateUy = false, size_t csrFloats = 0, bool mix = false) {
+  FusedShape s;
+  s.NB = NB, s.layoutJ = J, s.liveJ = J, s.P = P, s.U = U, s.nsrc = nsrc, s.n = n, s.numCells = numCells, s.cellsBehindRho = cellsBehindRho;
+  s.GT = GT, s.genRows = genRows, s.separateUy = separateUy, s.csrFloats = csrFloats, s.mix = mix;
+  return fusedLayout(s);
+}
+
+MMX_HD inline int fusedResidentMask(const FusedLayout& l) {
+  return (l.payloadFloats > 0 ? 1 : 0) | (l.rowRecWords > 0 ? 2 : 0);
+}
+
+}
diff --git a/momentum_amd/csrc/mmx_kernels.hpp b/momentum_amd/csrc/mmx_kernels.hpp
--- a/momentum_amd/csrc/mmx_kernels.hpp
+++ b/momentum_amd/csrc/mmx_kernels.hpp
@@ -119,6 +119,7 @@
   int32_t GT, genRows;
   const int32_t* tileList;
   int32_t numTiles;
+  int32_t residentInputs;
 };
 
 struct FusedParams {
@@ -143,6 +144,7 @@
 };
 
 size_t fusedLdsBytes(int NB, int J, int P, int U, int nsrc, int n, int numCells, bool cellsBehindRho, int GT = 0, int genRows = 0, bool separateUy = false, size_t csrFloats = 0, bool mix = false);
+int fusedResidentInputs(const RigDev& rig, const ProblemDev& pb, const FusedDev& fd);
 size_t fusedCsrFloats(int J, int nnz);
 size_t treeNormalEquationsLdsBytes(int J, int P, int U, int nsrc, int n, int GT = 0, int genRows = 0);
 size_t treeRefineLdsBytes(int J, int P, int U, int n, int genRows);
diff --git a/momentum_amd/csrc/mmx_mixed.hpp b/momentum_amd/csrc/mmx_mixed.hpp
--- a/momentum_amd/csrc/mmx_mixed.hpp
+++ b/momentum_amd/csrc/mmx_mixed.hpp
@@ -5,8 +5,6 @@
 
 namespace mmx {
 
-constexpr int kJsD = 17;
-constexpr int kTanD = 8;
 constexpr float kMixFactorDamping = 1e-6f;
 constexpr double kLn2D = 0.693147180559945309417232121458176568;
 
@@ -27,15 +25,6 @@
   int16_t* hi;
   int layoutJ;
 };
-__host__ __device__ inline size_t mixXDoubles(int J, int nsrc) {
-  return size_t(7 * J > nsrc ? 7 * J : nsrc);
-}
-__host__ __device__ inline size_t mixYDoubles(int J, int P) {
-  return size_t(kTanD * J > P ? kTanD * J : P);
-}
-__host__ __device__ inline size_t mixPersistentDoubles(int J, int P, int U, int NP) {
-  return size_t(P) + size_t(kJsD) * J + 7 * size_t(U) + 5 * size_t(NP);
-}
 
 __device__ __forceinline__ void mixSinCos(double x, double* sOut, double* cOut) {
   if (!(fabs(x) < 1e5)) {
diff --git a/momentum_amd/csrc/mmx_tree.hpp b/momentum_amd/csrc/mmx_tree.hpp
--- a/momentum_amd/csrc/mmx_tree.hpp
+++ b/momentum_amd/csrc/mmx_tree.hpp
@@ -13,9 +13,6 @@
   return F3{c.x * p[7], c.y * p[7], c.z * p[7]};
 }
 
-constexpr int kC2 = 17;
-constexpr int kC2Used = 16;
-constexpr int kC1 = 7;
 
 template <int NC, bool kSubtree, int STRIDE = NC, int UN = 1, class I = int32_t>
 __device__ __forceinline__ void treeSumT(
```

Result: no change. 2.228 million solves/s (-0.7%).
